# BillyXYB/TransEditor

Hardware: AMD Instinct MI355X
Metric: 256x256 images/sec/GPU, G+D fwd+bwd, batch 16; 1/2/4/8-GPU scaling (higher is better)
Workload: dtype f32

## Files before the change

include/te_hip.h:

```cpp
#ifndef TE_HIP_H
#define TE_HIP_H

#include <stdint.h>

#ifdef __cplusplus
extern "C" {
#endif

#define TE_ABI_VERSION 3

#define TE_ERR_NULL -1
#define TE_ERR_SHAPE -2
#define TE_ERR_UNSUPPORTED -3
#define TE_ERR_WORKSPACE -4

typedef void* te_stream_t;

int te_version(void);
const char* te_last_error_string(void);
const char* te_arch(void);

int te_bias_act_f32(float* out, const float* x, const float* b, const float* ref, int act, int grad,
                    float alpha, float scale, int64_t size_x, int64_t step_b, int64_t size_b,
                    te_stream_t stream);
int te_bias_act_f16(void* out, const void* x, const void* b, const void* ref, int act, int grad,
                    float alpha, float scale, int64_t size_x, int64_t step_b, int64_t size_b,
                    te_stream_t stream);
int te_bias_act_f64(double* out, const double* x, const double* b, const double* ref, int act, int grad,
                    float alpha, float scale, int64_t size_x, int64_t step_b, int64_t size_b,
                    te_stream_t stream);

int64_t te_bias_act_bwd_ws_floats(int64_t outer, int64_t C, int64_t inner);
int te_bias_act_bwd_f32(float* gi, float* gb, float* ws, const float* g, const float* ref, float alpha, float scale,
                        int64_t outer, int64_t C, int64_t inner, te_stream_t stream);
int te_bias_act_bwd_rgb_supported(int64_t outer, int64_t C, int64_t inner);
int te_bias_act_bwd_rgb_f32(float* gi, float* gb, float* ws, const float* g, const float* ref, const float* grgb, const float* wrgb,
                            const float* srgb, float wscale, float alpha, float scale, int64_t outer, int64_t C, int64_t inner,
                            te_stream_t stream);

int te_upfirdn2d_f32(float* out, const float* x, const float* k, int64_t major, int in_h, int in_w,
                     int minor, int kh, int kw, int up_x, int up_y, int down_x, int down_y, int pad_x0,
                     int pad_x1, int pad_y0, int pad_y1, const float* b, int64_t size_b, int act,
                     float alpha, float scale, te_stream_t stream);
int te_upfirdn2d_f16(void* out, const void* x, const void* k, int64_t major, int in_h, int in_w,
                     int minor, int kh, int kw, int up_x, int up_y, int down_x, int down_y, int pad_x0,
                     int pad_x1, int pad_y0, int pad_y1, te_stream_t stream);
int te_upfirdn2d_f64(double* out, const double* x, const double* k, int64_t major, int in_h, int in_w,
                     int minor, int kh, int kw, int up_x, int up_y, int down_x, int down_y, int pad_x0,
                     int pad_x1, int pad_y0, int pad_y1, te_stream_t stream);


#define TE_CONV_3X3 0
#define TE_CONV_T2 1
#define TE_CONV_S2 2
#define TE_CONV_1X1 3
#define TE_CONV_3X3W 4
#define TE_CONV_3X3W6 5

#define TE_CONV_S2S6 6

#define TE_CONV_T2S6 7

#define TE_CONV_1X1S6 8
#define TE_CONV_KINDS 9

#define TE_PACK_FWD 0
#define TE_PACK_DGRAD 1
#define TE_PACK_SWAP 2
#define TE_PACK_WFWD 3
#define TE_PACK_WDGRAD 4
#define TE_PACK_W6FWD 5
#define TE_PACK_W6DGRAD 6
#define TE_PACK_S6FWD 7
#define TE_PACK_S6SWAP 8
#define TE_PACK_T6FWD 9
#define TE_PACK_T6SWAP 10
#define TE_PACK_P6FWD 11
#define TE_PACK_P6DGRAD 12
#define TE_PACK_KINDS 13

int64_t te_conv_packed_numel(int kind_pack, int Co, int Ci, int ksize);
int te_conv_pack_weights_f32(float* wp, const float* w, float wscale, int kind_pack, int Co, int Ci,
                             int ksize, te_stream_t stream);
int te_conv_pack_weights2_f32(float* wp_a, int kind_a, float* wp_b, int kind_b, const float* w, float wscale, int Co, int Ci,
                              int ksize, te_stream_t stream);

int te_conv_pack_weights_multi_f32(int n, float* const* wp, const float* const* w, const float* wscale, const int* kind_pack,
                                   const int* Co, const int* Ci, const int* ksize, te_stream_t stream);

int te_conv_f32(float* out, const float* in, const float* wp, const float* isc, const float* osc,
                const float* bias, int act, int kind, int B, int K, int M, int H, int W,
                te_stream_t stream);
int te_conv_splitk_count(int kind, int B, int K, int M, int H, int W);
int te_conv_wino_supported(int B, int K, int M, int H, int W);
int te_conv_wino6_supported(int B, int K, int M, int H, int W);
int te_conv_s2s6_supported(int B, int K, int M, int H, int W);
int te_conv_t2s6_supported(int B, int K, int M, int H, int W);
int te_conv_p1s6_supported(int B, int K, int M, int H, int W);
int te_conv_wino6_form(int form);
int te_conv_wino6_tiles_per_block(int n);
int te_conv_s2s6_form(int form);
int te_conv_t2s6_form(int form);
int64_t te_conv_t2s6_ws_floats(int B, int K, int H);
int te_conv_ws_f32(float* out, float* ws, const float* in, const float* wp, const float* isc, const float* osc,
                   const float* bias, int act, int kind, int B, int K, int M, int H, int W, te_stream_t stream);
int te_conv_res_f32(float* out, float* ws, const float* in, const float* wp, const float* isc, const float* osc,
                    const float* bias, const float* res, const float* mask_ref, float mask_gain, int act, int kind, int B,
                    int K, int M, int H, int W, te_stream_t stream);

int te_wgrad_slab_count(int kind, int B, int Co, int Ci, int H, int W);
int te_wgrad_pair_form(int kind, int Co, int Ci, int H, int W);
int te_wgrad_split_supported(int kind, int Co, int Ci, int H, int W);
int te_wgrad_split_bf16(int on);
int te_wgrad_t2_wide(int on);
enum { TE_WG6_FP32 = 0, TE_WG6_3X3 = 1, TE_WG6_3X3_PAIR = 2, TE_WG6_T2_WIDE = 3, TE_WG6_T2 = 4, TE_WG6_T2_MASKED = 5, TE_WG6_1X1 = 6 };
int te_wgrad6_form(int kind, int B, int Co, int Ci, int H, int W, int NB);
int te_wgrad_f32(float* slabs, const float* g, const float* x, int kind, int B, int Co, int Ci, int H,
                 int W, int S, te_stream_t stream);
int te_wgrad_group_plan(int kind, int B, int Co, int Ci, int H, int W, int* NB, int* S);
int te_wgrad_group_f32(float* slabs, const float* g, const float* x, int kind, int B, int Co, int Ci, int H, int W, int S, int NB,
                       te_stream_t stream);

int64_t te_wgrad_reduce_ws_floats(int B, int S, int Co, int Ci, int taps, int want_w, int want_isc, int want_osc);
int te_wgrad_reduce_f32(float* gw, float* gisc, float* gosc, float* ws, const float* slabs, const float* w,
                        float wscale, const float* isc, const float* osc, int B, int S, int Co, int Ci,
                        int taps, te_stream_t stream);

int te_rgb_supported(int M, int K, int HW);
int te_rgb_fwd_f32(float* out, const float* x, const float* w, const float* isc, const float* bias, float wscale, int B,
                   int K, int HW, te_stream_t stream);
int te_rgb_dgrad_f32(float* gx, const float* g, const float* w, const float* isc, float wscale, int B, int K, int HW,
                     te_stream_t stream);
int te_rgb_expand_f32(float* out, const float* x3, const float* w, const float* bias, int act, float wscale, int B, int K,
                      int HW, te_stream_t stream);
int te_rgb_wgrad_slab_count(int B, int K, int HW);
int te_rgb_wgrad_f32(float* slabs, const float* g, const float* x, int B, int K, int HW, int S, te_stream_t stream);
int te_rgb_wgrad_sum_f32(float* slabs, const float* g, const float* x, int B, int K, int HW, int S, te_stream_t stream);

int te_attn_fwd_f32(float* o, float* sim, const float* q, const float* k, const float* v, float scale,
                    int N, int G, int M, int L, int D, te_stream_t stream);
int te_attn_bwd_f32(float* gq, float* gk, float* gv, const float* go, const float* gsim_or_null,
                    const float* q, const float* k, const float* v, const float* sim, float scale, int N,
                    int G, int M, int L, int D, te_stream_t stream);

int te_blur_actgrad_tiles(int in_h, int in_w, int kh, int kw, int pad_x0, int pad_x1, int pad_y0, int pad_y1);
int te_blur_actgrad_f32(float* gx, float* partial, const float* g, const float* ref, const float* k, int64_t major, int in_h,
                        int in_w, int kh, int kw, int pad_x0, int pad_x1, int pad_y0, int pad_y1, float alpha, float scale,
                        te_stream_t stream);
int te_blur_gradact_f32(float* gx, float* partial, const float* g, const float* ref, const float* k, int64_t major, int in_h,
                        int in_w, int kh, int kw, int pad_x0, int pad_x1, int pad_y0, int pad_y1, float alpha, float scale,
                        te_stream_t stream);

int te_upfirdn2d_plan(int64_t major, int in_h, int in_w, int minor, int kh, int kw, int up_x, int up_y, int down_x, int down_y,
                      int pad_x0, int pad_x1, int pad_y0, int pad_y1, int* zgroups, int* tiles);
int te_blur_actgrad_plan(int64_t major, int in_h, int in_w, int kh, int kw, int pad_x0, int pad_x1, int pad_y0, int pad_y1,
                         int* zgroups, int* tiles);
int te_blur_gradact_plan(int64_t major, int in_h, int in_w, int kh, int kw, int pad_x0, int pad_x1, int pad_y0, int pad_y1,
                         int* zgroups, int* tiles);
int64_t te_upfirdn2d_direct_cover(int64_t outputs);
int64_t te_chan_scale_cover(int64_t rows, int64_t hw, int aligned16);
int64_t te_bias_act_f32_cover(int64_t size_x, int64_t step_b, int aligned16, int* vec);
int64_t te_bias_act_any_cover(int64_t size_x);
int64_t te_conv_finalize_cover(int64_t outputs);
int64_t te_small_gemm_splitk_finish_cover(int I, int J);
int te_conv_pack_plan(int kind_pack, int Co, int Ci, int ksize, int* blocks, int* tiles);
int te_wgrad_reduce_plan(int B, int S, int Co, int Ci, int taps, int* parts, int64_t* cover);

int te_small_gemm_f32(float* c, float* pre, const float* a, const float* b, const float* bias, const float* residual,
                      float* arowsum, float rs_scale, int I, int J, int K, int64_t sai, int64_t sak, int64_t sbk,
                      int64_t sbj, float alpha, float beta, int act, te_stream_t stream);

int te_small_gemm_splitk_f32(float* c, float* pre, float* ws, int S, const float* a, const float* b, const float* bias,
                             const float* residual, int I, int J, int K, int64_t sai, int64_t sak, int64_t sbk, int64_t sbj,
                             float alpha, float beta, int act, te_stream_t stream);

int te_minibatch_stddev_fwd_f32(float* y, const float* x, int B, int group, int C, int HW, float eps, te_stream_t stream);
int te_minibatch_stddev_bwd_f32(float* gx, const float* gy, const float* x, int B, int group, int C, int HW, float eps,
                                te_stream_t stream);

int te_layer_norm_supported(int64_t R, int N);
int te_layer_norm_fwd_f32(float* y, float* stats, const float* x, int64_t R, int N, float eps, te_stream_t stream);
int te_layer_norm_bwd_f32(float* gx, const float* g, const float* y, const float* stats, int64_t R, int N, te_stream_t stream);

int te_pixel_norm_supported(int64_t B, int D, int C);
int te_pixel_norm_fwd_f32(float* y, float* r, const float* x, int64_t B, int D, int C, float eps, te_stream_t stream);
int te_pixel_norm_bwd_f32(float* gx, const float* g, const float* y, const float* r, int64_t B, int D, int C, te_stream_t stream);

int te_small_gemm_batched_f32(float* c, const float* a, const float* b, const float* bias, int nz, int64_t za, int64_t zc,
                              int64_t zb, int64_t zbias, const int64_t* b_tab, const int64_t* bias_tab, int I, int J, int K,
                              int64_t sai, int64_t sak, int64_t sbk, int64_t sbj, int64_t sci, int64_t scj, float alpha,
                              float beta, int act, te_stream_t stream);

int te_demod_fwd_f32(float* d, float* wsq, const float* w, const float* s, float wscale, float eps, int B, int Co, int Ci,
                     int T, te_stream_t stream);
int te_demod_bwd_f32(float* gw, float* gs, const float* gd, const float* d, const float* w, const float* wsq,
                     const float* s, float wscale, int B, int Co, int Ci, int T, int accumulate, te_stream_t stream);

int te_mt_adam_f32(const int64_t* table, const int32_t* chunks, int n_tensors, int n_chunks, int chunk_elems, double lr,
                   double beta1, double beta2, double eps, int step, te_stream_t stream);
int te_mt_ema_f32(const int64_t* table, const int32_t* chunks, int n_tensors, int n_chunks, int chunk_elems, double decay,
                  te_stream_t stream);

int te_chan_scale_f32(float* out, const float* x, const float* s, int64_t rows, int64_t hw, te_stream_t stream);
int te_chan_dot_f32(float* out, const float* a, const float* b, int64_t rows, int64_t hw, te_stream_t stream);

int te_lpips_stem_fwd_f32(float* out, const float* x, const float* w, const float* b, int N, int H, int W, te_stream_t stream);
int te_lpips_stem_dgrad_f32(float* gx, const float* g, const float* y1, const float* w, int N, int H, int W, te_stream_t stream);
int te_maxpool2_fwd_f32(float* out, const float* x, int64_t planes, int H, int W, te_stream_t stream);
int te_maxpool2_bwd_f32(float* gx, const float* g, const float* x, int64_t planes, int H, int W, te_stream_t stream);
int te_lpips_normalize_f32(float* out, const float* x, int N, int C, int64_t HW, te_stream_t stream);
int te_lpips_head_blocks(int64_t HW);
int te_lpips_head_fwd_f32(float* partial, const float* f, const float* t, const float* w, int N, int Nt, int C, int64_t HW,
                          te_stream_t stream);
int te_lpips_dist_f32(float* d, const float* const* partial, const int64_t* hw, int L, int N, te_stream_t stream);
int te_lpips_head_bwd_f32(float* gf, const float* gin, const float* gd, const float* f, const float* t, const float* w, int N, int Nt,
                          int C, int64_t HW, int relu_mask, te_stream_t stream);
int te_lpips_pair_head_fwd_f32(float* partial, const float* f, const float* w, int N, int C, int64_t HW, te_stream_t stream);
int te_crop_resize_bilinear_f32(float* out, const float* img, int B, int H, int W, int y0, int x0, int hc, int wc, int h, int w,
                                te_stream_t stream);

int64_t te_noise_reg_ws_floats(const int* sizes, int n, int B);
int te_noise_reg_fwd_f32(float* loss, float* ws, float* const* maps, const int* sizes, int n, int B, te_stream_t stream);
int te_noise_reg_bwd_f32(float* const* grads, float* tws, const float* gloss, const float* ws, float* const* maps, const int* sizes,
                         int n, int B, te_stream_t stream);
int te_noise_normalize_f32(float* const* maps, const int* sizes, int n, int B, te_stream_t stream);

int64_t te_prdc_ws_bytes(int N, int M, int D, int k);
int te_row_sqnorm_f32(float* out, const float* x, int N, int D, te_stream_t stream);
int te_prdc_knn_f32(float* r2, const float* x, const float* nx, int N, int D, int k, void* ws, te_stream_t stream);
int te_prdc_counts_f32(int32_t* col_count, int32_t* row_any, float* row_min, const float* x, const float* nx, const float* rr2,
                       const float* y, const float* ny, const float* rf2, int N, int M, int D, void* ws, te_stream_t stream);

int te_vgg_stem_fwd_f32(float* out, const float* x, const float* w, const float* b, int N, int H, int W, te_stream_t stream);
int te_adaptive_avgpool_f32(float* out, const float* x, int64_t planes, int H, int W, int OH, int OW, te_stream_t stream);
int te_fc_stream_splits(int J, int K);
int64_t te_fc_stream_ws_bytes(int64_t I, int J, int K);
int te_fc_stream_f32(float* c, float* ws, const float* a, const float* w, const float* bias, int64_t I, int J, int K, int act,
                     te_stream_t stream);

int64_t te_fid_moments_ws_bytes(int64_t N, int D);
int te_fid_moments_f64(double* S, double* s, void* ws, const float* x, int64_t N, int D, int accumulate, te_stream_t stream);
int te_fid_finalize_f64(double* mean, double* cov, const double* S, const double* s, int64_t n, int D, te_stream_t stream);

int te_gram_f32(float* K, const float* x, int n, int D, te_stream_t stream);
int te_svm_smo_f64(double* alpha, double* rho, int32_t* info, const float* K, const int8_t* y, int n, double C, double eps,
                   int64_t max_iter, te_stream_t stream);
int te_svm_coef_f32(float* w, const float* x, const double* alpha, const int8_t* y, int n, int D, te_stream_t stream);

int te_conv2d_f32(float* out, const float* x, const float* w, const float* bias, int B, int Ci, int Co, int H, int W, int kh, int kw,
                  int s, int py, int px, int Ctot, int c0, int act, te_stream_t stream);
int te_pool3_f32(float* out, const float* x, int B, int C, int H, int W, int mode, int Ctot, int c0, te_stream_t stream);
int te_resize_bilinear_f32(float* out, const float* x, int64_t planes, int H, int W, int OH, int OW, te_stream_t stream);

int te_dex_stem_fwd_f32(float* out, const float* img, const float* w, const float* b, int N, int H, int W, int crop, te_stream_t stream);
int te_cls_score_f32(float* score, float* prob, const float* a, const float* w, const float* bias, int64_t I, int C, int K, int mode,
                     te_stream_t stream);

int te_attr_stem_fwd_f32(float* out, const float* img, const float* w, const float* b, int N, int S, int R, int C0, int preprocessed,
                         te_stream_t stream);
int te_avgpool2_act_f32(float* out, const float* x, int64_t planes, int H, int W, float slope, te_stream_t stream);
int te_attr_score_f32(float* logit, float* score, const float* a, const float* w, const float* bias, int64_t I, int K, float slope,
                      te_stream_t stream);

int te_conv2d_res_f32(float* out, const float* x, const float* w, const float* bias, const float* res, int B, int Ci, int Co, int H, int W,
                      int kh, int kw, int s, int py, int px, int act, te_stream_t stream);
int te_pose_stem_fwd_f32(float* out, const float* img, const float* w, const float* b, int N, int H, int W, int crop, int Co,
                         int preprocessed, te_stream_t stream);
int te_maxpool3s2p1_f32(float* out, const float* x, int64_t planes, int H, int W, te_stream_t stream);

int te_alex_stem_fwd_f32(float* out, const float* x, const float* w, const float* b, int N, int H, int W, int Co, te_stream_t stream);
int te_lpips_unit_f32(float* out, const float* f, int N, int C, int64_t HW, te_stream_t stream);
int64_t te_lpips_allpairs_ws_floats(int N, int C, int64_t HW);
int te_lpips_allpairs_fwd_f32(float* partial, const float* fh, const float* w, int N, int C, int64_t HW, te_stream_t stream);
int te_lpips_allpairs_dist_f32(float* D, const float* const* partial, const int* c, const int64_t* hw, int L, int N, te_stream_t stream);

int te_conv2d_prelu_f32(float* out, const float* x, const float* w, const float* bias, const float* slope, const float* in_scale,
                        const float* in_shift, int B, int Ci, int Co, int H, int W, int kh, int kw, int s, int py, int px, te_stream_t stream);
int te_id_stem_fwd_f32(float* out, const float* img, const float* w, const float* b, const float* slope, int N, int H, int W, int y0, int y1,
                       int x0, int x1, int Pn, int Co, te_stream_t stream);
int te_se_excite_f32(float* gate, const float* pooled, const float* w1, const float* w2, int B, int C, int R, te_stream_t stream);
int te_se_scale_add_f32(float* out, const float* res, const float* gate, const float* sc, int B, int C, int Ho, int Wo, int Hs, int Ws, int s,
                        te_stream_t stream);
int te_rows_unit_f32(float* out, const float* a, int64_t I, int D, te_stream_t stream);
int te_rows_dot_f32(float* out, const float* a, const float* b, int64_t I, int D, te_stream_t stream);

int te_conv2d_prelu_keep_f32(float* out, float* pre, const float* x, const float* w, const float* bias, const float* slope,
                             const float* in_scale, const float* in_shift, int B, int Ci, int Co, int H, int W, int kh, int kw, int s, int py,
                             int px, te_stream_t stream);
int te_id_stem_keep_f32(float* out, float* pre, const float* img, const float* w, const float* b, const float* slope, int N, int H, int W,
                        int y0, int y1, int x0, int x1, int Pn, int Co, te_stream_t stream);
int te_conv2d_dgrad_f32(float* gx, const float* g, const float* wt, const float* pre, const float* slope, const float* in_scale,
                        const float* add, int B, int Ci, int Co, int H, int W, int kh, int kw, int s, int py, int px, int add_s,
                        te_stream_t stream);
int te_se_bwd_f32(float* gr, float* ws, const float* gout, const float* r, const float* gate, const float* pooled, const float* w1,
                  const float* w2, int B, int C, int R, int Ho, int Wo, te_stream_t stream);
int te_id_stem_bwd_f32(float* gimg, float* ws, const float* g, const float* wt, const float* pre, const float* slope, int N, int H, int W,
                       int y0, int y1, int x0, int x1, int Pn, int Co, te_stream_t stream);
int te_rows_unit_bwd_f32(float* ga, const float* ge, const float* e, const float* a, int64_t I, int D, te_stream_t stream);

int te_conv2d_heads_splits(int Ci, int kh, int kw, int Ho, int Wo);
int64_t te_conv2d_heads_ws_bytes(int64_t B, int G, int Cg, int Ci, int kh, int kw, int Ho, int Wo);
int te_conv2d_heads_f32(float* out, float* ws, int64_t ws_bytes, const float* x, const float* w, const float* bias, int B, int G, int Ci,
                        int Cg, int H, int W, int kh, int kw, int s, int py, int px, int Ctot, int c0, int shared, float slope, int splits,
                        te_stream_t stream);
int te_upsample_add_f32(float* out, const float* x, const float* y, int64_t planes, int h, int w, int H, int W, te_stream_t stream);
int te_psp_codes_f32(float* z, float* p, const float* lat, const float* A, const float* bz, const float* z_avg, const float* p_avg,
                     int64_t B, int Ns, int Np, int D, int T, te_stream_t stream);

#ifdef __cplusplus
}
#endif
#endif
```

transeditor_amd/_lib.py:

```python
import ctypes as C
import os

import torch

from . import _abi

_HERE = os.path.dirname(os.path.abspath(__file__))
LIB_PATH = os.path.join(_HERE, 'libte_hip.so')
HEADER_PATH = os.path.join(_HERE, '..', 'include', 'te_hip.h')
_lib = _protos = None

CONV_3X3, CONV_T2, CONV_S2, CONV_1X1, CONV_3X3W, CONV_3X3W6, CONV_S2S6, CONV_T2S6, CONV_1X1S6 = 0, 1, 2, 3, 4, 5, 6, 7, 8
(PACK_FWD, PACK_DGRAD, PACK_SWAP, PACK_WFWD, PACK_WDGRAD, PACK_W6FWD, PACK_W6DGRAD, PACK_S6FWD, PACK_S6SWAP, PACK_T6FWD,
 PACK_T6SWAP, PACK_P6FWD, PACK_P6DGRAD) = range(13)


def _header_text():
    if not os.path.exists(HEADER_PATH):
        raise RuntimeError(f'{HEADER_PATH} is missing: the bindings of libte_hip.so are read from it')
    with open(HEADER_PATH) as f:
        return f.read()


def _prototypes():
    global _protos
    if _protos is None:
        text = _header_text()
        _protos = _abi.parse(text), _abi.abi_version(text)
    return _protos


def __getattr__(name):
    if name == 'EXPORTS':
        return tuple(_prototypes()[0])
    raise AttributeError(f'module {__name__!r} has no attribute {name!r}')


def lib():
    global _lib
    if _lib is None:
        if not os.path.exists(LIB_PATH):
            raise RuntimeError(f'{LIB_PATH} is missing: build it with `python -m transeditor_amd.build` '
                               '(there is no CPU / PyTorch fallback for the TransEditor hot path)')
        protos, version = _prototypes()
        L = C.CDLL(LIB_PATH)
        for name, (res, args) in protos.items():
            if not hasattr(L, name):
                raise RuntimeError(f'{LIB_PATH} does not export {name}')
            fn = getattr(L, name)
            fn.restype, fn.argtypes = res, args
        if L.te_arch() != b'gfx950':
            raise RuntimeError('libte_hip.so was not built for gfx950')
        if L.te_version() != version:
            raise RuntimeError(f'{LIB_PATH} has ABI version {L.te_version()} but include/te_hip.h declares {version}: '
                               'a stale library, rebuild it with `python -m transeditor_amd.build`')
        _lib = L
    return _lib


def _check(rc, what):
    if rc != 0:
        raise RuntimeError(f'{what} failed (code {rc}): {lib().te_last_error_string().decode()}')


def _launch(name, *args):
    rc = getattr(_lib or lib(), name)(*args, _stream())
    if rc:
        _check(rc, name)


_OPS = []


def _op(fn):
    _OPS.append(fn)
    return fn


_cur_dev = getattr(torch._C, '_cuda_getDevice', torch.cuda.current_device)


def _on_current_device(t):
    if t.device.index != _cur_dev():
        raise RuntimeError(f'te_hip: tensor on {t.device} but the current device is cuda:{torch.cuda.current_device()}; '
                           f'call torch.cuda.set_device (one process per GPU) or wrap the call in torch.cuda.device(...)')


def _ptr(t, dtype=torch.float32, dense=True):
    if t is None:
        return None
    if not (t.is_cuda and t.dtype == dtype and (t.is_contiguous() or not dense)):
        name = 'fp32' if dtype == torch.float32 else dtype
        raise RuntimeError(f'te_hip: expected {"a contiguous" if dense else "an"} {name} tensor on the GPU, got {t.dtype} {t.device} '
                           + (f'contiguous={t.is_contiguous()} ' if dense else '') + '(no CPU path exists)')
    _on_current_device(t)
    return t.data_ptr()


_ptr_as = _ptr


def _raw(t):
    return _ptr(t, dense=False)


def _stream():
    return torch.cuda.current_stream().cuda_stream


def _aligned16(t):
    if t is None or t.data_ptr() % 16 == 0:
        return t
    return t.clone(memory_format=torch.contiguous_format)


_OTHER = {torch.float16: 'f16', torch.float64: 'f64'}


def _dispatch(x):
    return (_OTHER[x.dtype], x.dtype) if x.dtype in _OTHER else ('f32', torch.float32)


def _inner(shape):
    n = 1
    for d in shape[2:]:
        n *= d
    return n


@_op
def bias_act(x, b, ref, act, grad, alpha, scale):
    x = x.contiguous()
    sfx, dt = _dispatch(x)
    out = torch.empty_like(x)
    _launch('te_bias_act_' + sfx, _ptr(out, dt), _ptr(x, dt), _ptr(b, dt), _ptr(ref, dt), act, grad, alpha, scale, x.numel(),
            _inner(x.shape), b.numel() if b is not None else 1)
    return out


def _bias_grad_buffers(want_bias, outer, Cn, inner, device):
    if not want_bias:
        return None, None
    n = lib().te_bias_act_bwd_ws_floats(outer, Cn, inner)
    return (torch.empty(Cn, device=device, dtype=torch.float32),
            torch.empty(n, device=device, dtype=torch.float32) if n > 0 else None)


@_op
def bias_act_bwd(g, ref, alpha, scale, want_bias=True):
    g = g.contiguous()
    if g.dtype in _OTHER:
        gi = bias_act(g, None, ref, 3, 1, alpha, scale)
        return gi, (gi.sum(dim=[0] + list(range(2, gi.ndim))) if want_bias else None)
    gi = torch.empty_like(g)
    Cn, inner = g.shape[1], _inner(g.shape)
    gb, ws = _bias_grad_buffers(want_bias, g.shape[0], Cn, inner, g.device)
    _launch('te_bias_act_bwd_f32', _ptr(gi), _ptr(gb), _ptr(ws), _ptr(g), _ptr(ref), alpha, scale, g.shape[0], Cn, inner)
    return gi, gb


def bias_act_bwd_rgb_supported(shape):
    return bool(lib().te_bias_act_bwd_rgb_supported(shape[0], shape[1], _inner(shape)))


@_op
def bias_act_bwd_rgb(g, ref, grgb, wrgb, srgb, wscale, alpha, scale, want_bias=True):
    ref, grgb = _aligned16(ref.contiguous()), _aligned16(grgb.contiguous())
    g = _aligned16(g.contiguous()) if g is not None else None
    gi = torch.empty_like(ref)
    Cn, inner = ref.shape[1], _inner(ref.shape)
    gb, ws = _bias_grad_buffers(want_bias, ref.shape[0], Cn, inner, ref.device)
    _launch('te_bias_act_bwd_rgb_f32', _ptr(gi), _ptr(gb), _ptr(ws), _ptr(g), _ptr(ref), _ptr(grgb), _ptr(wrgb.contiguous()),
            _ptr(srgb.contiguous()) if srgb is not None else None, wscale, alpha, scale, ref.shape[0], Cn, inner)
    return gi, gb


@_op
def upfirdn2d_raw(x, k, up, down, pad, bias=None, act=0, alpha=0.2, scale=1.0):
    x = x.contiguous()
    B, Cn, H, W = x.shape
    kh, kw = k.shape
    px0, px1, py0, py1 = pad
    oh = (H * up[1] + py0 + py1 - kh) // down[1] + 1
    ow = (W * up[0] + px0 + px1 - kw) // down[0] + 1
    if oh <= 0 or ow <= 0:
        raise RuntimeError(f'upfirdn2d: empty output {oh}x{ow}')
    out = torch.empty(B, Cn, oh, ow, device=x.device, dtype=x.dtype)
    sfx, dt = _dispatch(x)
    if sfx != 'f32':
        if bias is not None or act:
            raise RuntimeError('upfirdn2d: the fused bias / activation epilogue exists in fp32 only')
        k = k.to(dt)
    args = [_ptr(out, dt), _ptr(x, dt), _ptr(k.contiguous(), dt), B * Cn, H, W, 1, kh, kw, up[0], up[1], down[0], down[1],
            px0, px1, py0, py1]
    if sfx == 'f32':
        args += [_ptr(bias), bias.numel() if bias is not None else 1, act, alpha, scale]
    _launch('te_upfirdn2d_' + sfx, *args)
    return out


@_op
def blur_actgrad(g, ref, k_flipped, pad, alpha, scale):
    g, ref = g.contiguous(), ref.contiguous()
    B, Cn, H, W = g.shape
    kh, kw = k_flipped.shape
    px0, px1, py0, py1 = pad
    tiles = lib().te_blur_actgrad_tiles(H, W, kh, kw, px0, px1, py0, py1)
    if tiles <= 0:
        raise RuntimeError(f'te_blur_actgrad_tiles failed ({tiles})')
    gx = torch.empty(B, Cn, H + py0 + py1 - kh + 1, W + px0 + px1 - kw + 1, device=g.device, dtype=g.dtype)
    partial = torch.empty(B, Cn, tiles, device=g.device, dtype=g.dtype)
    _launch('te_blur_actgrad_f32', _ptr(gx), _ptr(partial), _ptr(g), _ptr(ref), _ptr(k_flipped.contiguous()), B * Cn, H, W, kh, kw, px0,
            px1, py0, py1, alpha, scale)
    return gx, partial.sum(dim=(0, 2))


@_op
def blur_gradact(g, ref, k_flipped, pad, alpha, scale):
    g, ref = g.contiguous(), ref.contiguous()
    B, Cn, H, W = g.shape
    kh, kw = k_flipped.shape
    px0, px1, py0, py1 = pad
    oh, ow = H + py0 + py1 - kh + 1, W + px0 + px1 - kw + 1
    if tuple(ref.shape) != (B, Cn, oh, ow):
        raise RuntimeError(f'blur_gradact: ref {tuple(ref.shape)} is not the shape of the adjoint blur output {(B, Cn, oh, ow)}')
    tiles = lib().te_blur_actgrad_tiles(H, W, kh, kw, px0, px1, py0, py1)
    if tiles <= 0:
        raise RuntimeError(f'te_blur_actgrad_tiles failed ({tiles})')
    gx = torch.empty(B, Cn, oh, ow, device=g.device, dtype=g.dtype)
    partial = torch.empty(B, Cn, tiles, device=g.device, dtype=g.dtype)
    _launch('te_blur_gradact_f32', _ptr(gx), _ptr(partial), _ptr(g), _ptr(ref), _ptr(k_flipped.contiguous()), B * Cn, H, W, kh, kw, px0,
            px1, py0, py1, alpha, scale)
    return gx, partial.sum(dim=(0, 2))


@_op
def conv_pack(w, kind_pack, wscale=1.0):
    w = w.contiguous()
    Co, Ci, ks, _ = w.shape
    n = lib().te_conv_packed_numel(kind_pack, Co, Ci, ks)
    wp = torch.empty(n, device=w.device, dtype=w.dtype)
    _launch('te_conv_pack_weights_f32', _ptr(wp), _ptr(w), wscale, kind_pack, Co, Ci, ks)
    return wp


@_op
def conv_pack2(w, kind_a, kind_b, wscale=1.0):
    w = w.contiguous()
    Co, Ci, ks, _ = w.shape
    wa = torch.empty(lib().te_conv_packed_numel(kind_a, Co, Ci, ks), device=w.device, dtype=w.dtype)
    wb = torch.empty(lib().te_conv_packed_numel(kind_b, Co, Ci, ks), device=w.device, dtype=w.dtype)
    _launch('te_conv_pack_weights2_f32', _ptr(wa), kind_a, _ptr(wb), kind_b, _ptr(w), wscale, Co, Ci, ks)
    return wa, wb


@_op
def conv_pack_multi(jobs):
    n = len(jobs)
    if not n:
        return
    for wp, w, _, _ in jobs:
        if not (w.is_contiguous() and wp.is_contiguous()):
            raise RuntimeError('te_hip: conv_pack_multi needs dense weights and buffers')
    arr = lambda ty, vals: (ty * n)(*vals)
    _launch('te_conv_pack_weights_multi_f32', n, arr(C.c_void_p, [_ptr(j[0]) for j in jobs]), arr(C.c_void_p, [_ptr(j[1]) for j in jobs]),
            arr(C.c_float, [float(j[3]) for j in jobs]), arr(C.c_int, [int(j[2]) for j in jobs]),
            arr(C.c_int, [j[1].shape[0] for j in jobs]), arr(C.c_int, [j[1].shape[1] for j in jobs]),
            arr(C.c_int, [j[1].shape[2] for j in jobs]))


def wino_ok(B, K, M, H, W):
    return bool(lib().te_conv_wino_supported(B, K, M, H, W))


def s2s6_ok(B, K, M, H, W):
    return bool(lib().te_conv_s2s6_supported(B, K, M, H, W))


def t2s6_ok(B, K, M, H, W):
    return bool(lib().te_conv_t2s6_supported(B, K, M, H, W))


def p1s6_ok(B, K, M, H, W):
    return bool(lib().te_conv_p1s6_supported(B, K, M, H, W))


def wino6_form(form=-1):
    return int(lib().te_conv_wino6_form(form))


def wino6_tiles_per_block(n=-1):
    return int(lib().te_conv_wino6_tiles_per_block(n))


def s2s6_form(form=-1):
    return int(lib().te_conv_s2s6_form(form))


def t2s6_form(form=-1):
    return int(lib().te_conv_t2s6_form(form))


def wino6_ok(B, K, M, H, W):
    return bool(lib().te_conv_wino6_supported(B, K, M, H, W))


def conv_out_shape(kind, B, M, H, W):
    if kind in (CONV_T2, CONV_T2S6):
        return (B, M, 2 * H + 1, 2 * W + 1)
    return (B, M, H, W)


@_op
def conv(x, wp, kind, M, H, W, isc=None, osc=None, bias=None, act=0, res=None, mask_ref=None, mask_gain=1.0):
    x = x.contiguous()
    if kind == CONV_1X1S6:
        x = _aligned16(x)
    res = _aligned16(res.contiguous()) if res is not None else None
    mask_ref = _aligned16(mask_ref.contiguous()) if mask_ref is not None else None
    B, K = x.shape[0], x.shape[1]
    out = torch.empty(conv_out_shape(kind, B, M, H, W), device=x.device, dtype=x.dtype)
    if res is not None and tuple(res.shape) != tuple(out.shape):
        raise RuntimeError(f'te_hip: residual {tuple(res.shape)} does not match the convolution output {tuple(out.shape)}')
    if mask_ref is not None and tuple(mask_ref.shape) != tuple(out.shape):
        raise RuntimeError(f'te_hip: mask reference {tuple(mask_ref.shape)} does not match the convolution output {tuple(out.shape)}')
    S = lib().te_conv_splitk_count(kind, B, K, M, H, W)
    if S < 1:
        raise RuntimeError(f'te_conv_splitk_count failed ({S})')
    ws = torch.empty((S,) + tuple(out.shape), device=x.device, dtype=x.dtype) if S > 1 else None
    if kind == CONV_T2S6:
        ws = torch.empty(B * K * H, device=x.device, dtype=x.dtype)
    _launch('te_conv_res_f32', _ptr(out), _ptr(ws), _ptr(x), _ptr(wp), _ptr(isc), _ptr(osc), _ptr(bias), _ptr(res), _ptr(mask_ref),
            mask_gain, act, kind, B, K, M, H, W)
    return out


@_op
def wgrad_slabs(g, x, kind, H, W, group=False):
    g, x = g.contiguous(), x.contiguous()
    B, Co, Ci = g.shape[0], g.shape[1], x.shape[1]
    taps = 1 if kind == CONV_1X1 else 9
    if group:
        nb, sc = C.c_int(0), C.c_int(0)
        _check(lib().te_wgrad_group_plan(kind, B, Co, Ci, H, W, C.byref(nb), C.byref(sc)), 'te_wgrad_group_plan')
        if nb.value > 1:
            slabs = torch.empty(B // nb.value, sc.value, Co, Ci, taps, device=g.device, dtype=g.dtype)
            _launch('te_wgrad_group_f32', _ptr(slabs), _ptr(g), _ptr(x), kind, B, Co, Ci, H, W, sc.value, nb.value)
            return slabs
    S = lib().te_wgrad_slab_count(kind, B, Co, Ci, H, W)
    if S <= 0:
        raise RuntimeError(f'te_wgrad_slab_count failed ({S})')
    slabs = torch.empty(B, S, Co, Ci, taps, device=g.device, dtype=g.dtype)
    _launch('te_wgrad_f32', _ptr(slabs), _ptr(g), _ptr(x), kind, B, Co, Ci, H, W, S)
    return slabs


def wgrad_t2_wide(on=-1):
    return int(lib().te_wgrad_t2_wide(on))


def wgrad_split(on=-1):
    return int(lib().te_wgrad_split_bf16(on))


def wgrad_split_ok(kind, Co, Ci, H, W):
    return bool(lib().te_wgrad_split_supported(kind, Co, Ci, H, W))


WGRAD6_FORMS = ('fp32', 'w6', 'w6pair', 't2wide', 't2narrow', 't2masked', 'p1')


def wgrad6_form(kind, B, Co, Ci, H, W, NB=1):
    return WGRAD6_FORMS[lib().te_wgrad6_form(kind, B, Co, Ci, H, W, NB)]


def wgrad_pair_form(kind, Co, Ci, H, W):
    return bool(lib().te_wgrad_pair_form(kind, Co, Ci, H, W))


@_op
def wgrad_reduce(slabs, w, wscale=1.0, isc=None, osc=None, want_w=True, want_isc=False, want_osc=False):
    B, S, Co, Ci, taps = slabs.shape
    dev, dt = slabs.device, slabs.dtype
    gw = torch.empty(Co, Ci, taps, device=dev, dtype=dt) if want_w else None
    gisc = torch.empty(B, Ci, device=dev, dtype=dt) if want_isc else None
    gosc = torch.empty(B, Co, device=dev, dtype=dt) if want_osc else None
    n = lib().te_wgrad_reduce_ws_floats(B, S, Co, Ci, taps, int(want_w), int(want_isc), int(want_osc))
    if n < 0:
        raise RuntimeError(f'te_wgrad_reduce_ws_floats failed ({n})')
    ws = torch.empty(n, device=dev, dtype=dt) if n > 0 else None
    _launch('te_wgrad_reduce_f32', _ptr(gw), _ptr(gisc), _ptr(gosc), _ptr(ws), _ptr(slabs), _ptr(w.contiguous()), wscale, _ptr(isc),
            _ptr(osc), B, S, Co, Ci, taps)
    return gw, gisc, gosc


def rgb_supported(M, K, HW):
    return bool(lib().te_rgb_supported(M, K, HW))


@_op
def rgb_fwd(x, w, isc, bias, wscale=1.0):
    x = _aligned16(x.contiguous())
    B, K, H, W = x.shape
    out = torch.empty(B, 3, H, W, device=x.device, dtype=x.dtype)
    _launch('te_rgb_fwd_f32', _ptr(out), _ptr(x), _ptr(w.contiguous()), _ptr(isc), _ptr(bias), wscale, B, K, H * W)
    return out


@_op
def rgb_dgrad(g, w, isc, K, wscale=1.0):
    g = _aligned16(g.contiguous())
    B, _, H, W = g.shape
    gx = torch.empty(B, K, H, W, device=g.device, dtype=g.dtype)
    _launch('te_rgb_dgrad_f32', _ptr(gx), _ptr(g), _ptr(w.contiguous()), _ptr(isc), wscale, B, K, H * W)
    return gx


@_op
def rgb_wgrad_sum_slabs(g3, x):
    g3, x = g3.contiguous(), x.contiguous()
    B, K, H, W = x.shape
    S = lib().te_rgb_wgrad_slab_count(B, K, H * W)
    slabs = torch.empty(B, S, 4, K, device=x.device, dtype=x.dtype)
    _launch('te_rgb_wgrad_sum_f32', _ptr(slabs), _ptr(g3), _ptr(x), B, K, H * W, S)
    return slabs


@_op
def rgb_expand(x3, w3k, bias, act, wscale=1.0):
    x3 = _aligned16(x3.contiguous())
    B, _, H, W = x3.shape
    K = w3k.shape[1]
    out = torch.empty(B, K, H, W, device=x3.device, dtype=x3.dtype)
    _launch('te_rgb_expand_f32', _ptr(out), _ptr(x3), _ptr(w3k.contiguous()), _ptr(bias), act, wscale, B, K, H * W)
    return out


@_op
def rgb_wgrad_slabs(g, x):
    g, x = g.contiguous(), x.contiguous()
    B, K, H, W = x.shape
    S = lib().te_rgb_wgrad_slab_count(B, K, H * W)
    slabs = torch.empty(B, S, 3, K, 1, device=x.device, dtype=x.dtype)
    _launch('te_rgb_wgrad_f32', _ptr(slabs), _ptr(g), _ptr(x), B, K, H * W, S)
    return slabs


@_op
def small_gemm(I, J, K, a, sai, sak, b, sbk, sbj, bias=None, residual=None, alpha=1.0, beta=1.0, act=0, want_pre=False,
               rowsum_scale=None):
    c = torch.empty(I, J, device=a.device, dtype=a.dtype)
    pre = torch.empty_like(c) if want_pre else None
    rs = torch.empty(I, device=a.device, dtype=a.dtype) if rowsum_scale is not None else None
    _launch('te_small_gemm_f32', _ptr(c), _ptr(pre), _raw(a), _raw(b), _ptr(bias), _ptr(residual), _ptr(rs),
            rowsum_scale if rowsum_scale is not None else 0.0, I, J, K, sai, sak, sbk, sbj, alpha, beta, act)
    return c, pre, rs


@_op
def small_gemm_splitk(I, J, K, S, a, sai, sak, b, sbk, sbj, bias=None, residual=None, alpha=1.0, beta=1.0, act=0, want_pre=False):
    c = torch.empty(I, J, device=a.device, dtype=a.dtype)
    pre = torch.empty_like(c) if want_pre else None
    ws = torch.empty(S, I, J, device=a.device, dtype=a.dtype)
    _launch('te_small_gemm_splitk_f32', _ptr(c), _ptr(pre), _ptr(ws), S, _raw(a), _raw(b), _ptr(bias), _ptr(residual), I, J, K, sai, sak,
            sbk, sbj, alpha, beta, act)
    return c, pre


@_op
def minibatch_stddev_fwd(x, group, eps, chunks=1):
    x = x.contiguous()
    B, Cn, H, W = x.shape
    y = torch.empty(B, Cn + 1, H, W, device=x.device, dtype=x.dtype)
    Bc = B // chunks
    for c in range(chunks):
        _launch('te_minibatch_stddev_fwd_f32', _ptr(y[c * Bc:(c + 1) * Bc]), _ptr(x[c * Bc:(c + 1) * Bc]), Bc, group, Cn, H * W, eps)
    return y


@_op
def minibatch_stddev_bwd(gy, x, group, eps, chunks=1):
    gy = gy.contiguous()
    B, Cn, H, W = x.shape
    gx = torch.empty_like(x)
    Bc = B // chunks
    for c in range(chunks):
        sl = slice(c * Bc, (c + 1) * Bc)
        _launch('te_minibatch_stddev_bwd_f32', _ptr(gx[sl]), _ptr(gy[sl]), _ptr(x[sl]), Bc, group, Cn, H * W, eps)
    return gx


@_op
def small_gemm_batched(c, a, b, bias, nz, za, zc, I, J, K, sai, sak, sbk, sbj, sci, scj, zb=0, zbias=0, b_tab=None,
                       bias_tab=None, alpha=1.0, beta=1.0, act=0):
    bt = (C.c_int64 * nz)(*b_tab) if b_tab is not None else None
    bit = (C.c_int64 * nz)(*bias_tab) if bias_tab is not None else None
    _launch('te_small_gemm_batched_f32', _raw(c), _raw(a), _raw(b), _raw(bias), nz, za, zc, zb, zbias, bt, bit, I, J, K, sai, sak, sbk, sbj,
            sci, scj, alpha, beta, act)
    return c


def layer_norm_supported(R, N):
    return bool(lib().te_layer_norm_supported(R, N))


@_op
def layer_norm_fwd(x2, eps):
    R, N = x2.shape
    y = torch.empty_like(x2)
    stats = torch.empty(R, 2, device=x2.device, dtype=x2.dtype)
    _launch('te_layer_norm_fwd_f32', _ptr(y), _ptr(stats), _ptr(x2), R, N, eps)
    return y, stats


@_op
def layer_norm_bwd(g2, y2, stats):
    R, N = y2.shape
    gx = torch.empty_like(y2)
    _launch('te_layer_norm_bwd_f32', _ptr(gx), _ptr(g2), _ptr(y2), _ptr(stats), R, N)
    return gx


def pixel_norm_supported(B, D, Cn):
    return bool(lib().te_pixel_norm_supported(B, D, Cn))


@_op
def pixel_norm_fwd(x, eps):
    B, D, Cn = x.shape
    y = torch.empty_like(x)
    r = torch.empty(B, Cn, device=x.device, dtype=x.dtype)
    _launch('te_pixel_norm_fwd_f32', _ptr(y), _ptr(r), _ptr(x), B, D, Cn, eps)
    return y, r


@_op
def pixel_norm_bwd(g, y, r):
    B, D, Cn = y.shape
    gx = torch.empty_like(y)
    _launch('te_pixel_norm_bwd_f32', _ptr(gx), _ptr(g), _ptr(y), _ptr(r), B, D, Cn)
    return gx


@_op
def demod_fwd(w, s, wscale, eps):
    Co, Ci, T = w.shape
    B = s.shape[0]
    d = torch.empty(B, Co, device=w.device, dtype=w.dtype)
    wsq = torch.empty(Co, Ci, device=w.device, dtype=w.dtype)
    _launch('te_demod_fwd_f32', _ptr(d), _ptr(wsq), _ptr(w), _ptr(s), wscale, eps, B, Co, Ci, T)
    return d, wsq


@_op
def demod_from_wsq(wsq, s, eps):
    Co, Ci = wsq.shape
    B = s.shape[0]
    d = torch.empty(B, Co, device=wsq.device, dtype=wsq.dtype)
    _launch('te_demod_fwd_f32', _ptr(d), None, _ptr(wsq), _ptr(s), 1.0, eps, B, Co, Ci, 0)
    return d


@_op
def demod_bwd(gd, d, w, wsq, s, wscale, want_w=True, want_s=True, into=None):
    Co, Ci, T = w.shape
    B = s.shape[0]
    if into is not None:
        gw, gs = into
    else:
        gw = torch.empty_like(w) if want_w else None
        gs = torch.empty_like(s) if want_s else None
    _launch('te_demod_bwd_f32', _ptr(gw), _ptr(gs), _ptr(gd.contiguous()), _ptr(d), _ptr(w), _ptr(wsq), _ptr(s), wscale, B, Co, Ci, T,
            1 if into is not None else 0)
    return gw, gs


@_op
def attn_fwd(q, k, v, scale, groups):
    q, k, v = q.contiguous(), k.contiguous(), v.contiguous()
    N, M, Cn = q.shape
    L = k.shape[1]
    D = Cn // groups
    o = torch.empty_like(q)
    sim = torch.empty(N, groups, M, L, device=q.device, dtype=q.dtype)
    _launch('te_attn_fwd_f32', _ptr(o), _ptr(sim), _ptr(q), _ptr(k), _ptr(v), scale, N, groups, M, L, D)
    return o, sim


@_op
def attn_bwd(go, gsim, q, k, v, sim, scale, groups):
    N, M, Cn = q.shape
    L = k.shape[1]
    gq, gk, gv = torch.empty_like(q), torch.empty_like(k), torch.empty_like(v)
    _launch('te_attn_bwd_f32', _ptr(gq), _ptr(gk), _ptr(gv), _ptr(go.contiguous()), _ptr(gsim.contiguous()) if gsim is not None else None,
            _ptr(q), _ptr(k), _ptr(v), _ptr(sim), scale, N, groups, M, L, Cn // groups)
    return gq, gk, gv


@_op
def mt_adam(table, chunks, n_tensors, n_chunks, chunk_elems, lr, beta1, beta2, eps, step):
    _on_current_device(table)
    _launch('te_mt_adam_f32', table.data_ptr(), chunks.data_ptr(), n_tensors, n_chunks, chunk_elems, lr, beta1, beta2, eps, step)


@_op
def mt_ema(table, chunks, n_tensors, n_chunks, chunk_elems, decay):
    _on_current_device(table)
    _launch('te_mt_ema_f32', table.data_ptr(), chunks.data_ptr(), n_tensors, n_chunks, chunk_elems, float(decay))


@_op
def chan_scale(x, s):
    x, s = x.contiguous(), s.contiguous()
    rows = x.shape[0] * x.shape[1]
    out = torch.empty_like(x)
    _launch('te_chan_scale_f32', _ptr(out), _ptr(x), _ptr(s), rows, x.numel() // max(rows, 1))
    return out


@_op
def chan_dot(a, b):
    a, b = a.contiguous(), b.contiguous()
    rows = a.shape[0] * a.shape[1]
    out = torch.empty(a.shape[0], a.shape[1], device=a.device, dtype=a.dtype)
    _launch('te_chan_dot_f32', _ptr(out), _ptr(a), _ptr(b), rows, a.numel() // max(rows, 1))
    return out


@_op
def lpips_stem_fwd(x, w, b):
    x = x.contiguous()
    N, _, H, W = x.shape
    out = torch.empty(N, 64, H, W, device=x.device, dtype=x.dtype)
    _launch('te_lpips_stem_fwd_f32', _ptr(out), _ptr(x), _ptr(w), _ptr(b), N, H, W)
    return out


@_op
def lpips_stem_dgrad(g, y1, w):
    g = g.contiguous()
    N, _, H, W = g.shape
    gx = torch.empty(N, 3, H, W, device=g.device, dtype=g.dtype)
    _launch('te_lpips_stem_dgrad_f32', _ptr(gx), _ptr(g), _ptr(y1), _ptr(w), N, H, W)
    return gx


@_op
def maxpool2_fwd(x):
    x = x.contiguous()
    N, Cn, H, W = x.shape
    out = torch.empty(N, Cn, H // 2, W // 2, device=x.device, dtype=x.dtype)
    _launch('te_maxpool2_fwd_f32', _ptr(out), _ptr(x), N * Cn, H, W)
    return out


@_op
def maxpool2_bwd(g, x):
    g = g.contiguous()
    N, Cn, H, W = x.shape
    gx = torch.empty_like(x)
    _launch('te_maxpool2_bwd_f32', _ptr(gx), _ptr(g), _ptr(x), N * Cn, H, W)
    return gx


@_op
def lpips_normalize(x):
    x = x.contiguous()
    out = torch.empty_like(x)
    _launch('te_lpips_normalize_f32', _ptr(out), _ptr(x), x.shape[0], x.shape[1], x.shape[2] * x.shape[3])
    return out


@_op
def lpips_head_fwd(f, t_hat, w):
    f = f.contiguous()
    N, Cn, H, W = f.shape
    nb = lib().te_lpips_head_blocks(H * W)
    partial = torch.empty(N, nb, device=f.device, dtype=f.dtype)
    _launch('te_lpips_head_fwd_f32', _ptr(partial), _ptr(f), _ptr(t_hat), _ptr(w), N, t_hat.shape[0], Cn, H * W)
    return partial


@_op
def lpips_dist(partials, hws):
    L, N = len(partials), partials[0].shape[0]
    d = torch.empty(N, device=partials[0].device, dtype=torch.float32)
    ptrs = (C.c_void_p * L)(*[_ptr(p) for p in partials])
    hw = (C.c_int64 * L)(*hws)
    _launch('te_lpips_dist_f32', _ptr(d), ptrs, hw, L, N)
    return d


@_op
def lpips_head_bwd(gd, f, t_hat, w, gin=None, relu_mask=True):
    f = f.contiguous()
    N, Cn, H, W = f.shape
    gf = torch.empty_like(f)
    _launch('te_lpips_head_bwd_f32', _ptr(gf), _ptr(gin.contiguous()) if gin is not None else None, _ptr(gd.contiguous()), _ptr(f),
            _ptr(t_hat), _ptr(w), N, t_hat.shape[0], Cn, H * W, 1 if relu_mask else 0)
    return gf


@_op
def lpips_pair_head_fwd(f, w):
    if f.shape[0] % 2:
        raise RuntimeError(f'te_hip: the paired LPIPS head needs an even batch, got {f.shape[0]}')
    f = f.contiguous()
    N, Cn, H, W = f.shape[0] // 2, f.shape[1], f.shape[2], f.shape[3]
# ... 642 lines not shown
```

transeditor_amd/csrc/bias_act.hip:

```cpp
#include "te_common.h"
#include <hip/hip_fp16.h>

namespace {

__device__ __forceinline__ float act_one(float x, float r, int mode, float alpha) {
    switch (mode) {
        case 30: return x > 0.f ? x : x * alpha;
        case 31: return r > 0.f ? x : x * alpha;
        case 12:
        case 32: return 0.f;
        default: return x;
    }
}

__global__ __launch_bounds__(256) void bias_act_vec4_kernel(float4* __restrict__ out, const float4* __restrict__ x,
                                                            const float* __restrict__ b, const float4* __restrict__ ref,
                                                            int mode, float alpha, float scale, uint32_t n4,
                                                            uint32_t step_b4, uint32_t size_b) {
    const uint32_t stride = gridDim.x * blockDim.x;
    for (uint32_t i = blockIdx.x * blockDim.x + threadIdx.x; i < n4; i += stride) {
        float4 v = x[i];
        if (b) {
            const float bb = b[(i / step_b4) % size_b];
            v.x += bb; v.y += bb; v.z += bb; v.w += bb;
        }
        float4 r = make_float4(0.f, 0.f, 0.f, 0.f);
        if (ref) r = ref[i];
        float4 y;
        y.x = act_one(v.x, r.x, mode, alpha) * scale;
        y.y = act_one(v.y, r.y, mode, alpha) * scale;
        y.z = act_one(v.z, r.z, mode, alpha) * scale;
        y.w = act_one(v.w, r.w, mode, alpha) * scale;
        out[i] = y;
    }
}

__global__ __launch_bounds__(256) void bias_act_scalar_kernel(float* __restrict__ out, const float* __restrict__ x,
                                                              const float* __restrict__ b, const float* __restrict__ ref,
                                                              int mode, float alpha, float scale, int64_t n,
                                                              int64_t step_b, int64_t size_b) {
    const int64_t stride = (int64_t)gridDim.x * blockDim.x;
    for (int64_t i = (int64_t)blockIdx.x * blockDim.x + threadIdx.x; i < n; i += stride) {
        float v = x[i];
        if (b) v += b[(i / step_b) % size_b];
        const float r = ref ? ref[i] : 0.f;
        out[i] = act_one(v, r, mode, alpha) * scale;
    }
}

__device__ __forceinline__ float wave_sum(float v) {
#pragma unroll
    for (int off = 32; off > 0; off >>= 1) v += __shfl_down(v, off, 64);
    return v;
}

__device__ __forceinline__ float block_sum_256(float v, float* lds4) {
    v = wave_sum(v);
    const int lane = threadIdx.x & 63, wid = threadIdx.x >> 6;
    if (lane == 0) lds4[wid] = v;
    __syncthreads();
    return lds4[0] + lds4[1] + lds4[2] + lds4[3];
}

constexpr int kBwdVecPerThread = 4;
__global__ __launch_bounds__(256) void bias_act_bwd_rows_kernel(float4* __restrict__ gi, float* __restrict__ part,
                                                                const float4* __restrict__ g, const float4* __restrict__ ref,
                                                                float alpha, float scale, uint32_t C, uint32_t inner4) {
    __shared__ float lds4[4];
    const uint32_t c = blockIdx.y, n = blockIdx.z;
    const size_t row = ((size_t)n * C + c) * inner4;
    const uint32_t base = blockIdx.x * (256 * kBwdVecPerThread);
    float acc = 0.f;
#pragma unroll
    for (int it = 0; it < kBwdVecPerThread; ++it) {
        const uint32_t i = base + it * 256 + threadIdx.x;
        if (i < inner4) {
            const float4 gv = g[row + i], rv = ref[row + i];
            float4 o;
            o.x = gv.x * (rv.x > 0.f ? 1.f : alpha) * scale;
            o.y = gv.y * (rv.y > 0.f ? 1.f : alpha) * scale;
            o.z = gv.z * (rv.z > 0.f ? 1.f : alpha) * scale;
            o.w = gv.w * (rv.w > 0.f ? 1.f : alpha) * scale;
            gi[row + i] = o;
            acc += (o.x + o.y) + (o.z + o.w);
        }
    }
    if (part) {
        const float tot = block_sum_256(acc, lds4);
        if (threadIdx.x == 0) part[((size_t)c * gridDim.z + n) * gridDim.x + blockIdx.x] = tot;
    }
}

__global__ __launch_bounds__(64) void bias_parts_sum_kernel(float* __restrict__ gb, const float* __restrict__ part, uint32_t parts) {
    const float* p = part + (size_t)blockIdx.x * parts;
    float acc = 0.f;
    for (uint32_t j = threadIdx.x; j < parts; j += 64) acc += p[j];
    acc = wave_sum(acc);
    if (threadIdx.x == 0) gb[blockIdx.x] = acc;
}

__global__ __launch_bounds__(256) void bias_act_bwd_rgb_rows_kernel(float4* __restrict__ gi, float* __restrict__ part,
                                                                    const float4* __restrict__ g, const float4* __restrict__ ref,
                                                                    const float4* __restrict__ grgb, const float* __restrict__ wrgb,
                                                                    const float* __restrict__ srgb, float wscale, float alpha,
                                                                    float scale, uint32_t C, uint32_t inner4) {
    __shared__ float lds4[4];
    const uint32_t c = blockIdx.y, n = blockIdx.z;
    const size_t row = ((size_t)n * C + c) * inner4;
    const size_t rrow = (size_t)n * 3 * inner4;
    const float sc = (srgb ? srgb[(size_t)n * C + c] : 1.f) * wscale;
    const float c0 = sc * wrgb[c], c1 = sc * wrgb[C + c], c2 = sc * wrgb[2 * C + c];
    const uint32_t base = blockIdx.x * (256 * kBwdVecPerThread);
    float acc = 0.f;
#pragma unroll
    for (int it = 0; it < kBwdVecPerThread; ++it) {
        const uint32_t i = base + it * 256 + threadIdx.x;
        if (i < inner4) {
            const float4 rv = ref[row + i];
            const float4 r0 = grgb[rrow + i], r1 = grgb[rrow + inner4 + i], r2 = grgb[rrow + 2 * (size_t)inner4 + i];
            float4 gv = g ? g[row + i] : make_float4(0.f, 0.f, 0.f, 0.f);
            gv.x += c0 * r0.x + c1 * r1.x + c2 * r2.x;
            gv.y += c0 * r0.y + c1 * r1.y + c2 * r2.y;
            gv.z += c0 * r0.z + c1 * r1.z + c2 * r2.z;
            gv.w += c0 * r0.w + c1 * r1.w + c2 * r2.w;
            float4 o;
            o.x = gv.x * (rv.x > 0.f ? 1.f : alpha) * scale;
            o.y = gv.y * (rv.y > 0.f ? 1.f : alpha) * scale;
            o.z = gv.z * (rv.z > 0.f ? 1.f : alpha) * scale;
            o.w = gv.w * (rv.w > 0.f ? 1.f : alpha) * scale;
            gi[row + i] = o;
            acc += (o.x + o.y) + (o.z + o.w);
        }
    }
    if (part) {
        const float tot = block_sum_256(acc, lds4);
        if (threadIdx.x == 0) part[((size_t)c * gridDim.z + n) * gridDim.x + blockIdx.x] = tot;
    }
}

__global__ __launch_bounds__(256) void bias_act_bwd_chan_kernel(float* __restrict__ gi, float* __restrict__ gb,
                                                                const float* __restrict__ g, const float* __restrict__ ref,
                                                                float alpha, float scale, int64_t outer, int64_t C,
                                                                int64_t inner) {
    __shared__ float lds4[4];
    const int64_t c = blockIdx.x;
    const int64_t per = outer * inner;
    float acc = 0.f;
    for (int64_t e = threadIdx.x; e < per; e += 256) {
        const int64_t n = e / inner, i = e - n * inner;
        const int64_t idx = (n * C + c) * inner + i;
        const float o = g[idx] * (ref[idx] > 0.f ? 1.f : alpha) * scale;
        gi[idx] = o;
        acc += o;
    }
    if (gb) {
        const float tot = block_sum_256(acc, lds4);
        if (threadIdx.x == 0) gb[c] = tot;
    }
}

__global__ __launch_bounds__(256) void bias_act_bwd_2d_kernel(float* __restrict__ gi, float* __restrict__ gb,
                                                              const float* __restrict__ g, const float* __restrict__ ref,
                                                              float alpha, float scale, int64_t N, int64_t C) {
    const int64_t c = (int64_t)blockIdx.x * 256 + threadIdx.x;
    if (c >= C) return;
    float acc = 0.f;
    for (int64_t n = 0; n < N; ++n) {
        const int64_t idx = n * C + c;
        const float o = g[idx] * (ref[idx] > 0.f ? 1.f : alpha) * scale;
        gi[idx] = o;
        acc += o;
    }
    if (gb) gb[c] = acc;
}

inline int bias_act_grid(int64_t items) { return (int)std::min<int64_t>(te::cdiv(items, 256), te::kNumCU * 8); }
inline bool bias_act_vec(int64_t size_x, bool has_b, int64_t step_b, bool al16) {
    return (size_x % 4 == 0) && (!has_b || step_b % 4 == 0) && al16 && (size_x / 4 < (int64_t)0xFFFFFFFF);
}

template <typename T> struct AccOf { typedef T type; };
template <> struct AccOf<__half> { typedef float type; };

template <typename T>
__global__ __launch_bounds__(256) void bias_act_any_kernel(T* __restrict__ out, const T* __restrict__ x, const T* __restrict__ b,
                                                           const T* __restrict__ ref, int mode, float alpha_, float scale_,
                                                           int64_t n, int64_t step_b, int64_t size_b) {
    typedef typename AccOf<T>::type A;
    const A alpha = (A)(T)alpha_, scale = (A)(T)scale_;
    const int64_t stride = (int64_t)gridDim.x * blockDim.x;
    for (int64_t i = (int64_t)blockIdx.x * blockDim.x + threadIdx.x; i < n; i += stride) {
        A v = (A)x[i];
        if (b) v += (A)b[(i / step_b) % size_b];
        const A r = ref ? (A)ref[i] : (A)0;
        A y;
        switch (mode) {
            case 30: y = v > (A)0 ? v : v * alpha; break;
            case 31: y = r > (A)0 ? v : v * alpha; break;
            case 12:
            case 32: y = (A)0; break;
            default: y = v;
        }
        out[i] = (T)(y * scale);
    }
}

template <typename T>
int bias_act_any(T* out, const T* x, const T* b, const T* ref, int act, int grad, float alpha, float scale, int64_t size_x,
                 int64_t step_b, int64_t size_b, te_stream_t stream_, const char* what) {
    TE_REQUIRE(out && x, TE_ERR_NULL, "%s: out/x is NULL", what);
    TE_REQUIRE(size_x >= 0, TE_ERR_SHAPE, "%s: size_x < 0", what);
    TE_REQUIRE(!b || (step_b > 0 && size_b > 0), TE_ERR_SHAPE, "%s: bias given but step_b/size_b <= 0", what);
    if (size_x == 0) return 0;
    const int grid = bias_act_grid(size_x);
    bias_act_any_kernel<T><<<grid, 256, 0, (hipStream_t)stream_>>>(out, x, b, ref, act * 10 + grad, alpha, scale, size_x,
                                                                   b ? step_b : 1, b ? size_b : 1);
    return te::launch_status(what);
}

}

extern "C" int te_bias_act_f16(void* out, const void* x, const void* b, const void* ref, int act, int grad, float alpha,
                               float scale, int64_t size_x, int64_t step_b, int64_t size_b, te_stream_t stream) {
    return bias_act_any<__half>((__half*)out, (const __half*)x, (const __half*)b, (const __half*)ref, act, grad, alpha, scale,
                                size_x, step_b, size_b, stream, "te_bias_act_f16");
}

extern "C" int te_bias_act_f64(double* out, const double* x, const double* b, const double* ref, int act, int grad, float alpha,
                               float scale, int64_t size_x, int64_t step_b, int64_t size_b, te_stream_t stream) {
    return bias_act_any<double>(out, x, b, ref, act, grad, alpha, scale, size_x, step_b, size_b, stream, "te_bias_act_f64");
}

extern "C" int te_bias_act_f32(float* out, const float* x, const float* b, const float* ref, int act, int grad,
                               float alpha, float scale, int64_t size_x, int64_t step_b, int64_t size_b,
                               te_stream_t stream_) {
    TE_REQUIRE(out && x, TE_ERR_NULL, "te_bias_act_f32: out/x is NULL");
    TE_REQUIRE(size_x >= 0, TE_ERR_SHAPE, "te_bias_act_f32: size_x < 0");
    TE_REQUIRE(!b || (step_b > 0 && size_b > 0), TE_ERR_SHAPE, "te_bias_act_f32: bias given but step_b/size_b <= 0");
    if (size_x == 0) return 0;
    hipStream_t stream = (hipStream_t)stream_;
    const int mode = act * 10 + grad;
    const bool vec = bias_act_vec(size_x, b != nullptr, step_b, te::aligned16(out) && te::aligned16(x) && (!ref || te::aligned16(ref)));
    if (vec) {
        const uint32_t n4 = (uint32_t)(size_x / 4);
        const int grid = bias_act_grid(n4);
        bias_act_vec4_kernel<<<grid, 256, 0, stream>>>((float4*)out, (const float4*)x, b, (const float4*)ref, mode, alpha,
                                                       scale, n4, b ? (uint32_t)(step_b / 4) : 1u,
                                                       b ? (uint32_t)size_b : 1u);
    } else {
        const int grid = bias_act_grid(size_x);
        bias_act_scalar_kernel<<<grid, 256, 0, stream>>>(out, x, b, ref, mode, alpha, scale, size_x, b ? step_b : 1,
                                                         b ? size_b : 1);
    }
    return te::launch_status("te_bias_act_f32");
}

extern "C" int64_t te_bias_act_f32_cover(int64_t size_x, int64_t step_b, int aligned16_, int* vec_out) {
    if (size_x <= 0 || step_b < 0) return TE_ERR_SHAPE;
    const bool vec = bias_act_vec(size_x, step_b > 0, step_b, aligned16_ != 0);
    if (vec_out) *vec_out = vec ? 1 : 0;
    return (int64_t)bias_act_grid(vec ? size_x / 4 : size_x) * 256 * (vec ? 4 : 1);
}

extern "C" int64_t te_bias_act_any_cover(int64_t size_x) {
    return size_x > 0 ? (int64_t)bias_act_grid(size_x) * 256 : TE_ERR_SHAPE;
}

static bool bwd_rows_path(int64_t outer, int64_t C, int64_t inner) {
    return inner % 4 == 0 && inner >= 1024 && C <= 65535 && outer <= 65535;
}

extern "C" int64_t te_bias_act_bwd_ws_floats(int64_t outer, int64_t C, int64_t inner) {
    if (outer <= 0 || C <= 0 || inner <= 0 || !bwd_rows_path(outer, C, inner)) return 0;
    return C * outer * te::cdiv(inner / 4, 256 * kBwdVecPerThread);
}

extern "C" int te_bias_act_bwd_f32(float* gi, float* gb, float* ws, const float* g, const float* ref, float alpha, float scale,
                                   int64_t outer, int64_t C, int64_t inner, te_stream_t stream_) {
    TE_REQUIRE(gi && g && ref, TE_ERR_NULL, "te_bias_act_bwd_f32: gi/g/ref is NULL");
    TE_REQUIRE(outer >= 0 && C > 0 && inner > 0, TE_ERR_SHAPE, "te_bias_act_bwd_f32: bad dims");
    if (outer == 0) return 0;
    hipStream_t stream = (hipStream_t)stream_;
    if (inner == 1) {
        bias_act_bwd_2d_kernel<<<(int)te::cdiv(C, 256), 256, 0, stream>>>(gi, gb, g, ref, alpha, scale, outer, C);
    } else if (bwd_rows_path(outer, C, inner) && te::aligned16(gi) && te::aligned16(g) && te::aligned16(ref) && (!gb || ws)) {
        const uint32_t inner4 = (uint32_t)(inner / 4);
        dim3 grid((unsigned)te::cdiv(inner4, 256 * kBwdVecPerThread), (unsigned)C, (unsigned)outer);
        bias_act_bwd_rows_kernel<<<grid, 256, 0, stream>>>((float4*)gi, gb ? ws : nullptr, (const float4*)g, (const float4*)ref, alpha,
                                                           scale, (uint32_t)C, inner4);
        if (gb) bias_parts_sum_kernel<<<(int)C, 64, 0, stream>>>(gb, ws, (uint32_t)(grid.x * grid.z));
    } else {
        bias_act_bwd_chan_kernel<<<(int)C, 256, 0, stream>>>(gi, gb, g, ref, alpha, scale, outer, C, inner);
    }
    return te::launch_status("te_bias_act_bwd_f32");
}

extern "C" int te_bias_act_bwd_rgb_supported(int64_t outer, int64_t C, int64_t inner) {
    return (outer > 0 && C > 0 && bwd_rows_path(outer, C, inner)) ? 1 : 0;
}

extern "C" int te_bias_act_bwd_rgb_f32(float* gi, float* gb, float* ws, const float* g, const float* ref, const float* grgb,
                                       const float* wrgb, const float* srgb, float wscale, float alpha, float scale, int64_t outer,
                                       int64_t C, int64_t inner, te_stream_t stream_) {
    TE_REQUIRE(gi && ref && grgb && wrgb, TE_ERR_NULL, "te_bias_act_bwd_rgb_f32: gi/ref/grgb/wrgb is NULL");
    TE_REQUIRE(!gb || ws, TE_ERR_NULL, "te_bias_act_bwd_rgb_f32: the bias gradient needs the workspace (te_bias_act_bwd_ws_floats)");
    TE_REQUIRE(te_bias_act_bwd_rgb_supported(outer, C, inner), TE_ERR_UNSUPPORTED,
               "te_bias_act_bwd_rgb_f32: needs inner %% 4 == 0 and inner >= 1024 (use te_rgb_dgrad_f32 + te_bias_act_bwd_f32)");
    TE_REQUIRE(te::aligned16(gi) && (!g || te::aligned16(g)) && te::aligned16(ref) && te::aligned16(grgb), TE_ERR_UNSUPPORTED,
               "te_bias_act_bwd_rgb_f32: 16-byte aligned tensors required");
    const uint32_t inner4 = (uint32_t)(inner / 4);
    dim3 grid((unsigned)te::cdiv(inner4, 256 * kBwdVecPerThread), (unsigned)C, (unsigned)outer);
    hipStream_t stream = (hipStream_t)stream_;
    bias_act_bwd_rgb_rows_kernel<<<grid, 256, 0, stream>>>((float4*)gi, gb ? ws : nullptr, (const float4*)g, (const float4*)ref,
                                                          (const float4*)grgb, wrgb, srgb, wscale, alpha, scale, (uint32_t)C, inner4);
    if (gb) bias_parts_sum_kernel<<<(int)C, 64, 0, stream>>>(gb, ws, (uint32_t)(grid.x * grid.z));
    return te::launch_status("te_bias_act_bwd_rgb_f32");
}
```

transeditor_amd/csrc/conv_common.h:

```cpp
#pragma once
#include "te_common.h"
#include <stdlib.h>
#include <algorithm>

typedef float f32x16 __attribute__((ext_vector_type(16)));
typedef float f32x4 __attribute__((ext_vector_type(4)));

constexpr unsigned OOBH = 0x40000000u;

__device__ __forceinline__ __amdgpu_buffer_rsrc_t make_rsrc(const float* p, unsigned bytes) {
    return __builtin_amdgcn_make_buffer_rsrc((void*)p, 0, bytes, 0x00020000);
}
__device__ __forceinline__ float buf_load(__amdgpu_buffer_rsrc_t r, unsigned off) {
    return __builtin_bit_cast(float, __builtin_amdgcn_raw_buffer_load_b32(r, off, 0, 0));
}

constexpr int KPAD = 16;
constexpr int MPAD = 128;
constexpr int NTHREADS = 256;


int te_wino_launch(float* out, const float* in, const float* U, const float* isc, const float* osc, const float* bias, const float* res,
                   const float* mask_ref, float mask_gain, int act, int B, int K, int M, int H, int W, hipStream_t s);
int te_wino6_launch(float* out, const float* in, const float* U, const float* isc, const float* osc, const float* bias, const float* res,
                    const float* mask_ref, float mask_gain, int act, int B, int K, int M, int H, int W, hipStream_t s);
int te_s2s6_launch(float* out, const float* in, const float* U, const float* isc, const float* osc, const float* bias, const float* res,
                   const float* mask_ref, float mask_gain, int act, int B, int K, int M, int H, int W, hipStream_t s);
int te_t2s6_launch(float* out, const float* in, const float* U, const float* isc, const float* osc, const float* bias, int act,
                   int B, int K, int M, int H, int W, hipStream_t s, float* colbuf = nullptr);
int te_t2s6_edge_launch(float* out, const float* in, const float* wplain, const float* isc, const float* osc, const float* bias, int act,
                        int B, int K, int M, int H, int W, int Kp, int Mp, hipStream_t s, const float* colbuf = nullptr);
int te_p1s6_launch(float* out, const float* in, const float* U, const float* res, int B, int K, int M, int H, int W, hipStream_t s);
```

transeditor_amd/csrc/rgb.hip:

```cpp
#include "te_common.h"

namespace {

constexpr int KMAX = 512;
constexpr int NOUT = 3;

__global__ __launch_bounds__(256) void rgb_fwd_kernel(float* __restrict__ out, const float* __restrict__ x,
                                                      const float* __restrict__ w, const float* __restrict__ isc,
                                                      const float* __restrict__ bias, float wscale, int K, int HW) {
    __shared__ float ws[NOUT][KMAX];
    const int b = blockIdx.y, tid = threadIdx.x;
    for (int k = tid; k < K; k += 256) {
        const float s = (isc ? isc[(size_t)b * K + k] : 1.f) * wscale;
#pragma unroll
        for (int o = 0; o < NOUT; ++o) ws[o][k] = w[o * K + k] * s;
    }
    __syncthreads();
    const int HW4 = HW >> 2;
    const int p4 = blockIdx.x * 256 + tid;
    if (p4 >= HW4) return;
    const float4* xp = reinterpret_cast<const float4*>(x + (size_t)b * K * HW) + p4;
    float4 acc[NOUT];
#pragma unroll
    for (int o = 0; o < NOUT; ++o) acc[o] = make_float4(0.f, 0.f, 0.f, 0.f);
#pragma unroll 8
    for (int k = 0; k < K; ++k) {
        const float4 v = xp[(size_t)k * HW4];
#pragma unroll
        for (int o = 0; o < NOUT; ++o) {
            const float c = ws[o][k];
            acc[o].x += c * v.x; acc[o].y += c * v.y; acc[o].z += c * v.z; acc[o].w += c * v.w;
        }
    }
#pragma unroll
    for (int o = 0; o < NOUT; ++o) {
        const float bb = bias ? bias[o] : 0.f;
        acc[o].x += bb; acc[o].y += bb; acc[o].z += bb; acc[o].w += bb;
        reinterpret_cast<float4*>(out + ((size_t)b * NOUT + o) * HW)[p4] = acc[o];
    }
}

__global__ __launch_bounds__(256) void rgb_dgrad_kernel(float* __restrict__ gx, const float* __restrict__ g,
                                                        const float* __restrict__ w, const float* __restrict__ isc,
                                                        float wscale, int K, int HW, const float* __restrict__ bias = nullptr,
                                                        int act = 0) {
    __shared__ float ws[NOUT][KMAX];
    const int b = blockIdx.y, tid = threadIdx.x;
    for (int k = tid; k < K; k += 256) {
        const float s = (isc ? isc[(size_t)b * K + k] : 1.f) * wscale;
#pragma unroll
        for (int o = 0; o < NOUT; ++o) ws[o][k] = w[o * K + k] * s;
    }
    __syncthreads();
    const int HW4 = HW >> 2;
    const int p4 = blockIdx.x * 256 + tid;
    if (p4 >= HW4) return;
    float4 gv[NOUT];
#pragma unroll
    for (int o = 0; o < NOUT; ++o) gv[o] = reinterpret_cast<const float4*>(g + ((size_t)b * NOUT + o) * HW)[p4];
    float4* op = reinterpret_cast<float4*>(gx + (size_t)b * K * HW) + p4;
    const float gain = act == 3 ? 1.4142135623730951f : 1.f;
#pragma unroll 4
    for (int k = 0; k < K; ++k) {
        const float c0 = ws[0][k], c1 = ws[1][k], c2 = ws[2][k];
        const float bb = bias ? bias[k] : 0.f;
        float4 r;
        r.x = c0 * gv[0].x + c1 * gv[1].x + c2 * gv[2].x + bb;
        r.y = c0 * gv[0].y + c1 * gv[1].y + c2 * gv[2].y + bb;
        r.z = c0 * gv[0].z + c1 * gv[1].z + c2 * gv[2].z + bb;
        r.w = c0 * gv[0].w + c1 * gv[1].w + c2 * gv[2].w + bb;
        if (act >= 3) {
            r.x = (r.x > 0.f ? r.x : 0.2f * r.x) * gain; r.y = (r.y > 0.f ? r.y : 0.2f * r.y) * gain;
            r.z = (r.z > 0.f ? r.z : 0.2f * r.z) * gain; r.w = (r.w > 0.f ? r.w : 0.2f * r.w) * gain;
        }
        op[(size_t)k * HW4] = r;
    }
}

inline int rgb_pow2(int v) { int p = 1; while (p < v) p <<= 1; return p; }
inline int rgb_tile_px(int K) { return std::max(32, std::min(256, 8192 / rgb_pow2(K))); }

template <bool SUM>
__global__ __launch_bounds__(256) void rgb_wgrad_kernel(float* __restrict__ slabs, const float* __restrict__ g,
                                                        const float* __restrict__ x, int K, int HW, int S, int TPX, int lgTPX, int K2) {
    constexpr int NROW = SUM ? NOUT + 1 : NOUT;
    extern __shared__ __attribute__((aligned(16))) float smem[];
    float* xl = smem;
    float* gl = smem + K * (TPX + 1);
    const int b = blockIdx.y, c = blockIdx.x, tid = threadIdx.x;
    const int ntile = (HW + TPX - 1) / TPX;
    const int t0 = (int)((int64_t)ntile * c / S), t1 = (int)((int64_t)ntile * (c + 1) / S);
    const float* xb = x + (size_t)b * K * HW;
    const float* gb = g + (size_t)b * NOUT * HW;
    const bool vec4 = (HW & 3) == 0 && ((reinterpret_cast<uintptr_t>(x) & 15) == 0);
    const int parts = K2 >= 256 ? 1 : 256 / K2;
    const int kk = K2 >= 256 ? tid : (tid & (K2 - 1)), part = K2 >= 256 ? 0 : tid / K2;
    const int nh = K2 > 256 ? 2 : 1;
    float acc[2][NOUT + 1] = {{0.f, 0.f, 0.f, 0.f}, {0.f, 0.f, 0.f, 0.f}};
    for (int tl = t0; tl < t1; ++tl) {
        const int p0 = tl * TPX;
        __syncthreads();
        if (vec4) {
            for (int e0 = 0; e0 < K * TPX; e0 += 256 * 8 * 4) {
                float4 st[8];
#pragma unroll
                for (int j = 0; j < 8; ++j) {
                    const int e = e0 + 4 * (tid + 256 * j), k = e >> lgTPX, pp = e & (TPX - 1);
                    const bool ok = e < K * TPX && p0 + pp < HW;
                    st[j] = ok ? *reinterpret_cast<const float4*>(xb + (size_t)k * HW + p0 + pp) : make_float4(0.f, 0.f, 0.f, 0.f);
                }
#pragma unroll
                for (int j = 0; j < 8; ++j) {
                    const int e = e0 + 4 * (tid + 256 * j), k = e >> lgTPX, pp = e & (TPX - 1);
                    if (e < K * TPX) {
                        float* d = xl + k * (TPX + 1) + pp;
                        d[0] = st[j].x; d[1] = st[j].y; d[2] = st[j].z; d[3] = st[j].w;
                    }
                }
            }
        } else {
            for (int e0 = 0; e0 < K * TPX; e0 += 256 * 8) {
                float st[8];
#pragma unroll
                for (int j = 0; j < 8; ++j) {
                    const int e = e0 + tid + 256 * j, k = e >> lgTPX, pp = e & (TPX - 1);
                    const bool ok = e < K * TPX && p0 + pp < HW;
                    const float v = xb[ok ? (size_t)k * HW + p0 + pp : 0];
                    st[j] = ok ? v : 0.f;
                }
#pragma unroll
                for (int j = 0; j < 8; ++j) {
                    const int e = e0 + tid + 256 * j, k = e >> lgTPX, pp = e & (TPX - 1);
                    if (e < K * TPX) xl[k * (TPX + 1) + pp] = st[j];
                }
            }
        }
        for (int e = tid; e < NOUT * TPX; e += 256) {
            const int o = e >> lgTPX, pp = e & (TPX - 1);
            gl[e] = (p0 + pp < HW) ? gb[(size_t)o * HW + p0 + pp] : 0.f;
        }
        __syncthreads();
        for (int h = 0; h < nh; ++h) {
            const int k = kk + 256 * h;
            if (k < K) {
#pragma unroll 4
                for (int pp = part; pp < TPX; pp += parts) {
                    const float xv = xl[k * (TPX + 1) + pp];
#pragma unroll
                    for (int o = 0; o < NOUT; ++o) acc[h][o] += gl[o * TPX + pp] * xv;
                    if (SUM) acc[h][NOUT] += xv;
                }
            }
        }
    }
    float* sl = slabs + ((size_t)b * S + c) * NROW * K;
    if (parts > 1) {
        __syncthreads();
        float* red = smem;
#pragma unroll
        for (int o = 0; o < NROW; ++o) red[(part * NROW + o) * K2 + kk] = acc[0][o];
        __syncthreads();
        if (part == 0 && kk < K) {
#pragma unroll
            for (int o = 0; o < NROW; ++o) {
                float a = 0.f;
                for (int q = 0; q < parts; ++q) a += red[(q * NROW + o) * K2 + kk];
                sl[o * K + kk] = a;
            }
        }
        return;
    }
    for (int h = 0; h < nh; ++h) {
        const int k = kk + 256 * h;
        if (k < K) {
#pragma unroll
            for (int o = 0; o < NROW; ++o) sl[o * K + k] = acc[h][o];
        }
    }
}

inline bool ok_shape(int K, int HW) { return K > 0 && K <= KMAX && HW > 0 && (HW & 3) == 0; }

}

extern "C" int te_rgb_supported(int M, int K, int HW) { return (M == NOUT && ok_shape(K, HW)) ? 1 : 0; }

extern "C" int te_rgb_fwd_f32(float* out, const float* x, const float* w, const float* isc, const float* bias, float wscale,
                              int B, int K, int HW, te_stream_t stream_) {
    TE_REQUIRE(out && x && w, TE_ERR_NULL, "te_rgb_fwd_f32: NULL pointer");
    TE_REQUIRE(B > 0 && ok_shape(K, HW), TE_ERR_UNSUPPORTED, "te_rgb_fwd_f32: need K <= 512 and H*W %% 4 == 0");
    dim3 grid((unsigned)te::cdiv(HW / 4, 256), (unsigned)B);
    rgb_fwd_kernel<<<grid, 256, 0, (hipStream_t)stream_>>>(out, x, w, isc, bias, wscale, K, HW);
    return te::launch_status("te_rgb_fwd_f32");
}

extern "C" int te_rgb_dgrad_f32(float* gx, const float* g, const float* w, const float* isc, float wscale, int B, int K,
                                int HW, te_stream_t stream_) {
    TE_REQUIRE(gx && g && w, TE_ERR_NULL, "te_rgb_dgrad_f32: NULL pointer");
    TE_REQUIRE(B > 0 && ok_shape(K, HW), TE_ERR_UNSUPPORTED, "te_rgb_dgrad_f32: need K <= 512 and H*W %% 4 == 0");
    dim3 grid((unsigned)te::cdiv(HW / 4, 256), (unsigned)B);
    rgb_dgrad_kernel<<<grid, 256, 0, (hipStream_t)stream_>>>(gx, g, w, isc, wscale, K, HW);
    return te::launch_status("te_rgb_dgrad_f32");
}

extern "C" int te_rgb_expand_f32(float* out, const float* x3, const float* w, const float* bias, int act, float wscale, int B,
                                 int K, int HW, te_stream_t stream_) {
    TE_REQUIRE(out && x3 && w, TE_ERR_NULL, "te_rgb_expand_f32: NULL pointer");
    TE_REQUIRE(B > 0 && ok_shape(K, HW), TE_ERR_UNSUPPORTED, "te_rgb_expand_f32: need K <= 512 and H*W %% 4 == 0");
    TE_REQUIRE(act == 0 || act == 3 || act == 4, TE_ERR_UNSUPPORTED, "te_rgb_expand_f32: act must be 0, 3 or 4");
    dim3 grid((unsigned)te::cdiv(HW / 4, 256), (unsigned)B);
    rgb_dgrad_kernel<<<grid, 256, 0, (hipStream_t)stream_>>>(out, x3, w, nullptr, wscale, K, HW, bias, act);
    return te::launch_status("te_rgb_expand_f32");
}

extern "C" int te_rgb_wgrad_slab_count(int B, int K, int HW) {
    if (B <= 0 || K <= 0 || HW <= 0) return TE_ERR_SHAPE;
    const int64_t ntile = te::cdiv(HW, rgb_tile_px(K));
    int64_t S = te::cdiv(4 * te::kNumCU, B);
    return (int)std::max<int64_t>(1, std::min<int64_t>(S, ntile));
}

extern "C" int te_rgb_wgrad_f32(float* slabs, const float* g, const float* x, int B, int K, int HW, int S, te_stream_t stream_) {
    TE_REQUIRE(slabs && g && x, TE_ERR_NULL, "te_rgb_wgrad_f32: NULL pointer");
    TE_REQUIRE(B > 0 && K > 0 && K <= KMAX && HW > 0 && S > 0, TE_ERR_UNSUPPORTED, "te_rgb_wgrad_f32: need 0 < K <= 512");
    const int TPX = rgb_tile_px(K), K2 = rgb_pow2(K);
    int lg = 0;
    while ((1 << lg) < TPX) ++lg;
    const size_t lds = sizeof(float) * std::max<size_t>((size_t)K * (TPX + 1) + NOUT * TPX, (size_t)256 * (NOUT + 1));
    static std::atomic<uint64_t> attr_done{0};
    te::allow_big_lds(attr_done, (const void*)rgb_wgrad_kernel<false>, 96 * 1024);
    dim3 grid((unsigned)S, (unsigned)B);
    rgb_wgrad_kernel<false><<<grid, 256, lds, (hipStream_t)stream_>>>(slabs, g, x, K, HW, S, TPX, lg, K2);
    return te::launch_status("te_rgb_wgrad_f32");
}

extern "C" int te_rgb_wgrad_sum_f32(float* slabs, const float* g, const float* x, int B, int K, int HW, int S, te_stream_t stream_) {
    TE_REQUIRE(slabs && g && x, TE_ERR_NULL, "te_rgb_wgrad_sum_f32: NULL pointer");
    TE_REQUIRE(B > 0 && K > 0 && K <= KMAX && HW > 0 && S > 0, TE_ERR_UNSUPPORTED, "te_rgb_wgrad_sum_f32: need 0 < K <= 512");
    const int TPX = rgb_tile_px(K), K2 = rgb_pow2(K);
    int lg = 0;
    while ((1 << lg) < TPX) ++lg;
    const size_t lds = sizeof(float) * std::max<size_t>((size_t)K * (TPX + 1) + NOUT * TPX, (size_t)256 * (NOUT + 1));
    static std::atomic<uint64_t> attr_done{0};
    te::allow_big_lds(attr_done, (const void*)rgb_wgrad_kernel<true>, 96 * 1024);
    dim3 grid((unsigned)S, (unsigned)B);
    rgb_wgrad_kernel<true><<<grid, 256, lds, (hipStream_t)stream_>>>(slabs, g, x, K, HW, S, TPX, lg, K2);
    return te::launch_status("te_rgb_wgrad_sum_f32");
}
```

transeditor_amd/csrc/wino6.hip:

```cpp
#include "split6_common.h"
#include "wino6_schedule.h"
#ifdef W6P_PROF
#define TE_PROF
#endif
#include "te_prof.h"

namespace {

constexpr int WT = 512, KC = 16, TW = 32, NP = TW / 2, BM = 64, TH = 8;
constexpr int U_CHUNKS = 36 * 2 * 64;

struct Wino6Args {
    float* out; const float* in; const u32x4* U; const float* isc; const float* osc; const float* bias; const float* res;
    const float* mref; float mgain; int act;
    int B, K, M, H, W, ntiles, mblocks, tiles_x, tiles_y, nt8;
    int lists;
    int lgpw;
};

constexpr int PH = 4, PR = PH + 2;
constexpr int TP_PLANE = PR * 2 * NP * 4;
constexpr int TP_DWORDS = 12 * TP_PLANE;
constexpr int GT = WT / 2;
constexpr int P_IN = (PR * NP * 8) / GT;
static_assert(PR * NP * 8 == P_IN * GT, "items must divide over the group");

PROF_BUFFER(w6p, 2048 * 8 * 8)
constexpr int SLOT0 = 21;

template <bool ISC>
__global__ __launch_bounds__(WT, 2) void wino6p_kernel(const Wino6Args p) {
    extern __shared__ __attribute__((aligned(16))) unsigned char smem_raw[];
    u32x4* ul = reinterpret_cast<u32x4*>(smem_raw);
    const int tid = threadIdx.x, lane = tid & 63, l31 = lane & 31, half = lane >> 5;
    const int wid = __builtin_amdgcn_readfirstlane(tid >> 6);
    const int grp = wid >> 2, wq = wid & 3, wm = wq >> 1, wrl = wq & 1, gt = tid & (GT - 1);
    unsigned* tl = reinterpret_cast<unsigned*>(smem_raw + U_CHUNKS * 16) + grp * TP_DWORDS;
    const u32x4* tl4 = reinterpret_cast<const u32x4*>(tl);
    int tile, mb;
    if (!split6_tile(p.ntiles, p.nt8, p.mblocks, tile, mb)) return;
    const int pwm = (1 << p.lgpw) - 1;
    const int tx = tile % p.tiles_x, ty = (tile / p.tiles_x) % p.tiles_y, b = (tile / (p.tiles_x * p.tiles_y)) << (4 - p.lgpw);
    const int x0 = tx * TW, y0 = ty * TH, yh = y0 + PH * grp;
    const float* inb = p.in + (size_t)b * p.K * p.H * p.W;
    const float* iscb = ISC ? p.isc + (size_t)b * p.K : nullptr;
    const bool has_left = x0 == 0, has_right = x0 + TW >= p.W, has_rowout = (yh == 0) || (yh + PH == p.H);

    f32x16 acc[4];
#pragma unroll
    for (int c = 0; c < 4; ++c)
#pragma unroll
        for (int r = 0; r < 16; ++r) acc[c][r] = 0.f;

    unsigned g_off[P_IN];
    int l_off[P_IN], e_flag[P_IN];
#pragma unroll
    for (int i = 0; i < P_IN; ++i) {
        const int e = gt + GT * i;
        const int jj = e & 15, q = (e >> 4) & 7, row = e >> 7;
        const int gy = yh - 1 + row;
        const int sj = jj >> p.lgpw, jl = jj & pwm;
        const bool left = x0 == 0 && jl == 0, right = x0 + TW >= p.W && jl == pwm, rowout = gy < 0 || gy >= p.H;
        e_flag[i] = (left ? 1 : 0) | (right ? 2 : 0) | (rowout ? 4 : 0);
        const int gyc = gy < 0 ? 0 : (gy >= p.H ? p.H - 1 : gy);
        g_off[i] = (unsigned)(sj * p.K * p.H * p.W + (2 * q * p.H + gyc) * p.W + x0 + 2 * jl - 1 + (left ? 1 : 0) - (right ? 1 : 0));
        l_off[i] = ((row * 2 + (q >> 2)) * NP + jj) * 4 + (q & 3);
    }
    const unsigned q2 = 2u * ((gt >> 4) & 7) + (unsigned)(((gt & 15) >> p.lgpw) * p.K);
    const size_t plane = (size_t)p.H * p.W;
    const int MT = p.M >> 5;
    f32x4 rin[P_IN][2];
    f32x2 rsc = {1.f, 1.f};
    const int nstage = p.K / KC;
    auto fetch_scales = [&](int s) {
        if (ISC) rsc = *reinterpret_cast<const f32x2u*>(iscb + s * KC + q2);
    };
    auto fetch_item = [&](int i, int s) {
#pragma unroll
        for (int h2 = 0; h2 < 2; ++h2)
            rin[i][h2] = *reinterpret_cast<const f32x4u*>(inb + ((size_t)s * KC + h2) * plane + g_off[i]);
    };
    auto issue = [&](int s) {
        fetch_scales(s);
#pragma unroll
        for (int i = 0; i < P_IN; ++i) fetch_item(i, s);
    };
    auto issue_u = [&](int uh, int s) {
        const u32x4* us = p.U + (size_t)s * 36 * MT * 64;
#pragma unroll
        for (int r = 0; r < 9; ++r) {
            const int j = wq * 9 + r, piece = j / 12, rem = j % 12, kc = (rem >> 1) + 6 * uh, mt = rem & 1;
            const int pk = piece * 12 + kc;
            const u32x4* g = us + ((size_t)pk * MT + 2 * mb + mt) * 64 + (unsigned)lane;
            __builtin_amdgcn_global_load_lds((const __attribute__((address_space(1))) void*)g,
                                             (__attribute__((address_space(3))) void*)(ul + (pk * 2 + mt) * 64), 16, 0, 0);
        }
    };
    unsigned res[P_IN][4][3];
    float te = 0.f, to = 0.f, fe = 0.f, fo = 0.f;
    constexpr int N_SLOT = 3 + 4 * 4 * P_IN;
    auto arith = [&](int k) {
        if (k < 0) {
        } else if (k < P_IN) {
#pragma unroll
            for (int h2 = 0; h2 < 2; ++h2) {
                f32x4 v = rin[k][h2];
                const int f = e_flag[k];
                if (has_left) {
                    asm volatile("" ::: "memory");
                    if (f & 1) { v[3] = v[2]; v[2] = v[1]; v[1] = v[0]; v[0] = 0.f; }
                }
                if (has_right) {
                    asm volatile("" ::: "memory");
                    if (f & 2) { v[0] = v[1]; v[1] = v[2]; v[2] = v[3]; v[3] = 0.f; }
                }
                if (has_rowout) {
                    asm volatile("" ::: "memory");
                    if (f & 4) { v[0] = 0.f; v[1] = 0.f; v[2] = 0.f; v[3] = 0.f; }
                }
                rin[k][h2] = ISC ? v * rsc[h2] : v;
                asm volatile("" : "+v"(rin[k][h2]));
            }
        } else if (k < N_SLOT) {
            const int u = (k - P_IN) >> 2, j = (k - P_IN) & 3, i = u >> 2, c = u & 3;
            float ve = 0.f, vo = 0.f;
            if (j == 0) {
                const f32x4 e = rin[i][0], o = rin[i][1];
                ve = c == 0 ? e[0] - e[2] : (c == 1 ? e[1] + e[2] : (c == 2 ? e[2] - e[1] : e[1] - e[3]));
                vo = c == 0 ? o[0] - o[2] : (c == 1 ? o[1] + o[2] : (c == 2 ? o[2] - o[1] : o[1] - o[3]));
            }
            split6_step4(j, ve, vo, te, to, fe, fo, res[i][c][0], res[i][c][1], res[i][c][2]);
        }
    };
    auto write_res = [&]() {
#pragma unroll
        for (int i = 0; i < P_IN; ++i)
#pragma unroll
            for (int c = 0; c < 4; ++c)
#pragma unroll
                for (int pc = 0; pc < 3; ++pc) tl[l_off[i] + (pc * 4 + c) * TP_PLANE] = res[i][c][pc];
    };
    const int rr = l31 >> 4, jj = l31 & 15;
    const int b_chunk = ((2 * wrl + rr) * 2 + half) * NP + jj;
    const int a_chunk = wm * 64 + lane;

    issue(0);
    if (grp == 0) { issue_u(0, 0); issue_u(1, 0); }
#pragma unroll
    for (int k = 0; k < N_SLOT; ++k) arith(k);
    write_res();
    issue(1);
    if (grp == 0) {
        if (ISC) asm volatile("s_waitcnt vmcnt(7)" ::: "memory");
        else asm volatile("s_waitcnt vmcnt(6)" ::: "memory");
    }
    split6_barrier();
    const int nphase = 2 * nstage;
    PROF_ONLY(unsigned long long pc[8] = {0, 0, 0, 0, 0, 0, 0, 0};)
    PROF_ONLY(const unsigned long long pstart = __builtin_readcyclecounter(), rstart = __builtin_amdgcn_s_memrealtime();)
    for (int ph = 0; ph < nphase; ++ph) {
        const bool last = ph == nphase - 1;
        PROF_T(t0);
        if ((ph & 1) == grp) {
            bf16x8 av[2][3], bv[2][3];
            const int fs2 = min((ph >> 1) + 2, nstage - 1);
            auto rd1 = [&](int g, int slot, int q) {
                const int ky = g >> 2, c = g & 3;
                if (q < 3) av[slot][q] = __builtin_bit_cast(bf16x8, ul[a_chunk + ((q * 3 + ky) * 4 + c) * 128]);
                else bv[slot][q - 3] = __builtin_bit_cast(bf16x8, tl4[b_chunk + (((q - 3) * 4 + c) * PR + ky) * 2 * NP]);
            };
#pragma unroll
            for (int q = 0; q < 6; ++q) rd1(0, 0, q);
            __builtin_amdgcn_s_setprio(1);
#pragma unroll
            for (int g = 0; g < 12; ++g) {
                const int slot = g & 1, c = g & 3;
                if (g == 5) { PROF_T(ta); split6_barrier(); PROF_T(tb); PROF_ACC(pc[0], t0, ta); PROF_ACC(pc[1], ta, tb); PROF_ONLY(pc[2] -= tb;) }
                __builtin_amdgcn_sched_barrier(0);
#pragma unroll
                for (int q = 0; q < 6; ++q) {
                    split6_product(q, av[slot], bv[slot], acc[c], acc[c]);
                    if (g + 1 < 12 && q < 3) { rd1(g + 1, slot ^ 1, 2 * q); rd1(g + 1, slot ^ 1, 2 * q + 1); }
                    arith(g * 6 + q - SLOT0);
                    {
                        constexpr int LASTQ = 71 - SLOT0;
                        const int k = g * 6 + q - SLOT0;
                        if (k == P_IN - 1) fetch_scales(fs2);
#pragma unroll
                        for (int i = 0; i < P_IN; ++i)
                            if (k == (P_IN + 16 * i + 12 < LASTQ ? P_IN + 16 * i + 12 : LASTQ)) fetch_item(i, fs2);
                    }
                    __builtin_amdgcn_sched_barrier(0);
                }
            }
            __builtin_amdgcn_s_setprio(0);
            PROF_ONLY({ asm volatile("s_nop 0" ::: "memory"); PROF_T(tc); pc[2] += tc; })
        } else {
            const int cs = (ph + 1) >> 1;
            const bool work = cs >= 1 && cs < nstage;
            if (grp == 1 && work) issue_u(1, cs);
            __builtin_amdgcn_sched_barrier(0);
            write_res();
            if (grp == 1 && work) split6_wait_vm();
            PROF_T(ta);
            split6_barrier();
            PROF_T(tb);
            if (grp == 0 && work) {
                issue_u(0, cs);
                split6_wait_vm();
            }
            PROF_T(tc);
            PROF_ACC(pc[3], t0, ta); PROF_ACC(pc[4], ta, tb); PROF_ACC(pc[5], tb, tc);
        }
        PROF_T(t8);
        if (!last) split6_barrier();
        PROF_T(t9);
        PROF_ACC(pc[6], t8, t9);
    }
    PROF_ONLY(if (lane == 0 && blockIdx.x < 2048) {
        unsigned long long* d = te_w6p_prof_buf + ((size_t)blockIdx.x * 8 + wid) * 8;
        _Pragma("unroll")
        for (int i = 0; i < 6; ++i) d[i] = pc[i];
        d[6] = pc[6] | ((__builtin_amdgcn_s_memrealtime() - rstart) << 40);
        d[7] = ((unsigned long long)nstage << 48) | ((__builtin_readcyclecounter() - pstart) & 0xFFFFFFFFFFFFull);
    })
    const int wr = grp * 2 + wrl;
    const int mbase = mb * BM + wm * 32;
    const int bo = b + (jj >> p.lgpw);
    const size_t off0 = ((size_t)bo * p.M + mbase) * plane + (size_t)(y0 + 2 * wr + rr) * p.W + x0 + 2 * (jj & pwm);
    const float g_pos = p.act == 3 ? 1.4142135623730951f : 1.f;
    float scv[16], biv[16];
#pragma unroll
    for (int r = 0; r < 16; ++r) {
        const int m = mbase + (r & 3) + 8 * (r >> 2) + 4 * half;
        scv[r] = p.osc ? p.osc[(size_t)bo * p.M + m] : 1.f;
        biv[r] = p.bias ? p.bias[m] : 0.f;
    }
    f32x2 resv[16], mrefv[16];
    if (p.res) {
#pragma unroll
        for (int r = 0; r < 16; ++r)
            resv[r] = *reinterpret_cast<const f32x2*>(p.res + off0 + (size_t)((r & 3) + 8 * (r >> 2) + 4 * half) * plane);
    }
    if (p.mref) {
#pragma unroll
        for (int r = 0; r < 16; ++r)
            mrefv[r] = *reinterpret_cast<const f32x2*>(p.mref + off0 + (size_t)((r & 3) + 8 * (r >> 2) + 4 * half) * plane);
    }
#pragma unroll
    for (int r = 0; r < 16; ++r) {
        const int dm = (r & 3) + 8 * (r >> 2) + 4 * half;
        float v0 = acc[0][r] + acc[1][r] + acc[2][r];
        float v1 = acc[1][r] - acc[2][r] - acc[3][r];
        const float sc = scv[r], bi = biv[r];
        v0 = v0 * sc + bi;
        v1 = v1 * sc + bi;
        if (p.act >= 3) {
            v0 = (v0 > 0.f ? v0 : v0 * 0.2f) * g_pos;
            v1 = (v1 > 0.f ? v1 : v1 * 0.2f) * g_pos;
        }
        const size_t o = off0 + (size_t)dm * plane;
        if (p.res) { v0 += resv[r][0]; v1 += resv[r][1]; }
        if (p.mref) {
            v0 *= mrefv[r][0] > 0.f ? p.mgain : 0.2f * p.mgain;
            v1 *= mrefv[r][1] > 0.f ? p.mgain : 0.2f * p.mgain;
        }
        f32x2 v; v[0] = v0; v[1] = v1;
        *reinterpret_cast<f32x2*>(p.out + o) = v;
    }
}


template <bool ISC>
__global__ __launch_bounds__(WT, 2) void wino6q_kernel(const Wino6Args p) {
    extern __shared__ __attribute__((aligned(16))) unsigned char smem_raw[];
    u32x4* ul = reinterpret_cast<u32x4*>(smem_raw);
    const int tid = threadIdx.x, lane = tid & 63, l31 = lane & 31, half = lane >> 5;
    const int wid = __builtin_amdgcn_readfirstlane(tid >> 6);
    const int grp = wid >> 2, wq = wid & 3, wm = wq >> 1, wrl = wq & 1, gt = tid & (GT - 1);
    unsigned* tl = reinterpret_cast<unsigned*>(smem_raw + U_CHUNKS * 16) + grp * TP_DWORDS;
    const u32x4* tl4 = reinterpret_cast<const u32x4*>(tl);
    int tile, tile_end, tile_step, mbq;
    if (!split6_tile_list(p.ntiles, p.nt8, p.mblocks, p.lists, tile, tile_end, tile_step, mbq)) return;
    const float* inb;
    const float* iscb = nullptr;
    bool has_left, has_right, has_rowout;

    f32x16 acc[2][4];
#pragma unroll
    for (int m = 0; m < 2; ++m)
#pragma unroll
        for (int c = 0; c < 4; ++c)
#pragma unroll
            for (int r = 0; r < 16; ++r) acc[m][c][r] = 0.f;

    unsigned g_off[P_IN];
    int l_off[P_IN], e_flag[P_IN];
    typedef const __attribute__((address_space(4))) Wino6Args* KArgs;
    auto kargs = [&]() {
        KArgs k = (KArgs)__builtin_amdgcn_kernarg_segment_ptr();
        asm volatile("" : "+s"(k));
        return k;
    };
    auto set_tile = [&](int t) {
        const KArgs a = kargs();
        const int aH = a->H, aW = a->W, atx = a->tiles_x, aty = a->tiles_y, aK = a->K;
        const int tx = t % atx, ty = (t / atx) % aty, b = t / (atx * aty);
        const int x0 = tx * TW, yh = ty * TH + PH * grp;
        inb = a->in + (size_t)b * aK * aH * aW;
        if (ISC) iscb = a->isc + (size_t)b * aK;
        has_left = x0 == 0; has_right = x0 + TW == aW; has_rowout = (yh == 0) || (yh + PH == aH);
        int gto = gt;
        asm volatile("" : "+v"(gto));
#pragma unroll
        for (int i = 0; i < P_IN; ++i) {
            const int e = gto + GT * i;
            const int jj = e & 15, q = (e >> 4) & 7, row = e >> 7;
            const int gy = yh - 1 + row;
            const bool left = x0 == 0 && jj == 0, right = x0 + TW == aW && jj == NP - 1, rowout = gy < 0 || gy >= aH;
            e_flag[i] = (left ? 1 : 0) | (right ? 2 : 0) | (rowout ? 4 : 0);
            const int gyc = gy < 0 ? 0 : (gy >= aH ? aH - 1 : gy);
            g_off[i] = (unsigned)((2 * q * aH + gyc) * aW + x0 + 2 * jj - 1 + (left ? 1 : 0) - (right ? 1 : 0));
        }
    };
    set_tile(tile);
#pragma unroll
    for (int i = 0; i < P_IN; ++i) {
        const int e = gt + GT * i;
        const int jj = e & 15, q = (e >> 4) & 7, row = e >> 7;
        l_off[i] = ((row * 2 + (q >> 2)) * NP + jj) * 4 + (q & 3);
    }
    const unsigned q2 = 2u * ((gt >> 4) & 7);
    const size_t plane = (size_t)p.H * p.W;
    const int MT = p.M >> 5;
    f32x4 rin[P_IN][2];
    f32x2 rsc = {1.f, 1.f};
    const int nstage = p.K / KC, nimg = 2 * nstage;
    auto fetch_scales = [&](int s) {
        if (ISC) rsc = *reinterpret_cast<const f32x2u*>(iscb + s * KC + q2);
    };
    auto fetch_item = [&](int i, int s) {
#pragma unroll
        for (int h2 = 0; h2 < 2; ++h2)
            rin[i][h2] = *reinterpret_cast<const f32x4u*>(inb + ((size_t)s * KC + h2) * plane + g_off[i]);
    };
    auto issue_u = [&](int uh, int j) {
        int wqo = wq;
        asm volatile("" : "+s"(wqo));
        const u32x4* us = p.U + ((size_t)(j >> 1) * 36 * MT + 2 * (2 * mbq + (j & 1))) * 64;
        const unsigned pstride = 12u * (unsigned)MT * 64u;
#pragma unroll
        for (int t = 0; t < 3; ++t) {
            const int rem = wqo * 3 + t, kc = (rem >> 1) + 6 * uh, mt = rem & 1;
            const u32x4* g0 = us + (unsigned)(kc * MT + mt) * 64u;
            u32x4* l0 = ul + (kc * 2 + mt) * 64;
#pragma unroll
            for (int piece = 0; piece < 3; ++piece) {
                const u32x4* g = g0 + piece * pstride + (unsigned)lane;
                __builtin_amdgcn_global_load_lds((const __attribute__((address_space(1))) void*)g,
                                                 (__attribute__((address_space(3))) void*)(l0 + piece * 24 * 64), 16, 0, 0);
            }
        }
    };
    unsigned res[P_IN][4][3];
    float te = 0.f, to = 0.f, fe = 0.f, fo = 0.f;
    constexpr int N_SLOT = 3 + 4 * 4 * P_IN;
    auto arith = [&](int k) {
        if (k < 0) {
        } else if (k < P_IN) {
#pragma unroll
            for (int h2 = 0; h2 < 2; ++h2) {
                f32x4 v = rin[k][h2];
                if (has_left) {
                    int f = e_flag[k];
                    asm volatile("" : "+v"(f) :: "memory");
                    if (f & 1) { v[3] = v[2]; v[2] = v[1]; v[1] = v[0]; v[0] = 0.f; }
                }
                if (has_right) {
                    int f = e_flag[k];
                    asm volatile("" : "+v"(f) :: "memory");
                    if (f & 2) { v[0] = v[1]; v[1] = v[2]; v[2] = v[3]; v[3] = 0.f; }
                }
                if (has_rowout) {
                    int f = e_flag[k];
                    asm volatile("" : "+v"(f) :: "memory");
                    if (f & 4) { v[0] = 0.f; v[1] = 0.f; v[2] = 0.f; v[3] = 0.f; }
                }
                rin[k][h2] = ISC ? v * rsc[h2] : v;
                asm volatile("" : "+v"(rin[k][h2]));
            }
        } else if (k < N_SLOT) {
            const int u = (k - P_IN) >> 2, j = (k - P_IN) & 3, i = u >> 2, c = u & 3;
            float ve = 0.f, vo = 0.f;
            if (j == 0) {
                const f32x4 e = rin[i][0], o = rin[i][1];
                ve = c == 0 ? e[0] - e[2] : (c == 1 ? e[1] + e[2] : (c == 2 ? e[2] - e[1] : e[1] - e[3]));
                vo = c == 0 ? o[0] - o[2] : (c == 1 ? o[1] + o[2] : (c == 2 ? o[2] - o[1] : o[1] - o[3]));
            }
            split6_step4(j, ve, vo, te, to, fe, fo, res[i][c][0], res[i][c][1], res[i][c][2]);
        }
    };
    auto write_res = [&]() {
#pragma unroll
        for (int i = 0; i < P_IN; ++i)
#pragma unroll
            for (int c = 0; c < 4; ++c)
#pragma unroll
                for (int pc = 0; pc < 3; ++pc) tl[l_off[i] + (pc * 4 + c) * TP_PLANE] = res[i][c][pc];
    };
    const int rr = l31 >> 4, jj = l31 & 15;
    const int b_chunk = ((2 * wrl + rr) * 2 + half) * NP + jj;
    const int a_chunk = wm * 64 + lane;

    auto multiply = [&](auto mset_tag, int fs) {
        constexpr int MSET = decltype(mset_tag)::value;
        bf16x8 av[2][3], bv[2][3];
        auto rd1 = [&](int g, int slot, int q) {
            const int ky = g >> 2, c = g & 3;
            if (q < 3) av[slot][q] = __builtin_bit_cast(bf16x8, ul[a_chunk + ((q * 3 + ky) * 4 + c) * 128]);
            else bv[slot][q - 3] = __builtin_bit_cast(bf16x8, tl4[b_chunk + (((q - 3) * 4 + c) * PR + ky) * 2 * NP]);
        };
#pragma unroll
        for (int q = 0; q < 6; ++q) rd1(0, 0, q);
        __builtin_amdgcn_s_setprio(1);
#pragma unroll
        for (int g = 0; g < 12; ++g) {
            const int slot = g & 1, c = g & 3;
            if (g == 5) split6_barrier();
            __builtin_amdgcn_sched_barrier(0);
#pragma unroll
            for (int q = 0; q < 6; ++q) {
                split6_product(q, av[slot], bv[slot], acc[MSET][c], acc[MSET][c]);
                if (g + 1 < 12 && q < 3) { rd1(g + 1, slot ^ 1, 2 * q); rd1(g + 1, slot ^ 1, 2 * q + 1); }
                const int k = g * 6 + q;
                if (MSET == 0) {
                    if (k == 5) fetch_scales(fs);
#pragma unroll
                    for (int i = 0; i < P_IN; ++i)
                        if (k == 6 + 12 * i) fetch_item(i, fs);
                } else {
                    arith(k - SLOT0);
                }
                __builtin_amdgcn_sched_barrier(0);
            }
        }
        __builtin_amdgcn_s_setprio(0);
        split6_barrier();
    };
    auto stage = [&](int ph, bool write, bool has_next) {
        const int cs = wino6_sched::renew_image(ph);
        const bool work = wino6_sched::renew_work(cs, nimg, has_next);
        const int ci = cs == nimg ? 0 : cs;
        if (grp == 1 && work) issue_u(1, ci);
        __builtin_amdgcn_sched_barrier(0);
        if (write) write_res();
        if (grp == 1 && work) split6_wait_vm();
        split6_barrier();
        if (grp == 0 && work) {
            issue_u(0, ci);
            split6_wait_vm();
        }
        split6_barrier();
    };

    fetch_scales(0);
#pragma unroll
    for (int i = 0; i < P_IN; ++i) fetch_item(i, 0);
    if (grp == 0) { issue_u(0, 0); issue_u(1, 0); }
#pragma unroll
    for (int k = 0; k < N_SLOT; ++k) arith(k);
    write_res();
    split6_wait_vm();
    split6_barrier();
    for (;;) {
        const bool has_next = tile + tile_step < tile_end;
        int ph = 0;
        if (wino6_sched::lead_phase(grp)) { stage(0, false, has_next); ph = 1; }
        for (int s = 0; s < nstage; ++s) {
            bool next_tile;
            const int fs = wino6_sched::fetch_stage(s, nstage, has_next, next_tile);
            if (next_tile) set_tile(tile + tile_step);
            multiply(std::integral_constant<int, 0>{}, fs);
            stage(ph + 1, false, has_next);
            multiply(std::integral_constant<int, 1>{}, fs);
            if (wino6_sched::runs_sb(grp, s, nstage, has_next)) stage(ph + 3, true, has_next);
            ph += 4;
        }
        for (int i = 0; i < wino6_sched::tail_barriers(grp, has_next); ++i) split6_barrier();

        const KArgs e = kargs();
        const int tx = tile % e->tiles_x, ty = (tile / e->tiles_x) % e->tiles_y, b = tile / (e->tiles_x * e->tiles_y);
        const int x0 = tx * TW, y0 = ty * TH;
        int elane = lane;
        asm volatile("" : "+v"(elane));
        const int ehalf = elane >> 5, err = (elane & 31) >> 4, ejj = elane & 15;
        const int wr = grp * 2 + wrl;
        const int eM = e->M, eW = e->W, eact = e->act;
        const size_t eplane = (size_t)e->H * eW;
        const float emgain = e->mgain;
        const float g_pos = eact == 3 ? 1.4142135623730951f : 1.f;
        float* const eout = e->out;
        const float* const eosc = e->osc; const float* const ebias = e->bias; const float* const eres = e->res; const float* const emref = e->mref;
#pragma unroll
        for (int m = 0; m < 2; ++m) {
            const int mbase = (2 * mbq + m) * BM + wm * 32;
            const size_t off0 = ((size_t)b * eM + mbase) * eplane + (size_t)(y0 + 2 * wr) * eW + x0;
            const unsigned lo = (unsigned)(err * eW + 2 * ejj) + 4u * (unsigned)ehalf * (unsigned)eplane;
#pragma unroll
            for (int r0 = 0; r0 < 16; r0 += 4) {
                float scv[4], biv[4];
#pragma unroll
                for (int r = r0; r < r0 + 4; ++r) {
                    const int mm = mbase + (r & 3) + 8 * (r >> 2) + 4 * ehalf;
                    scv[r - r0] = eosc ? eosc[(size_t)b * eM + mm] : 1.f;
                    biv[r - r0] = ebias ? ebias[mm] : 0.f;
                }
                f32x2 resv[4], mrefv[4];
                if (eres) {
#pragma unroll
                    for (int r = r0; r < r0 + 4; ++r)
                        resv[r - r0] = *reinterpret_cast<const f32x2*>(eres + off0 + (size_t)((r & 3) + 8 * (r >> 2)) * eplane + lo);
                }
                if (emref) {
#pragma unroll
                    for (int r = r0; r < r0 + 4; ++r)
                        mrefv[r - r0] = *reinterpret_cast<const f32x2*>(emref + off0 + (size_t)((r & 3) + 8 * (r >> 2)) * eplane + lo);
                }
#pragma unroll
                for (int r = r0; r < r0 + 4; ++r) {
                    float v0 = acc[m][0][r] + acc[m][1][r] + acc[m][2][r];
                    float v1 = acc[m][1][r] - acc[m][2][r] - acc[m][3][r];
                    const float sc = scv[r - r0], bi = biv[r - r0];
                    v0 = v0 * sc + bi;
                    v1 = v1 * sc + bi;
                    if (eact >= 3) {
                        v0 = (v0 > 0.f ? v0 : v0 * 0.2f) * g_pos;
                        v1 = (v1 > 0.f ? v1 : v1 * 0.2f) * g_pos;
                    }
                    if (eres) { v0 += resv[r - r0][0]; v1 += resv[r - r0][1]; }
                    if (emref) {
                        v0 *= mrefv[r - r0][0] > 0.f ? emgain : 0.2f * emgain;
                        v1 *= mrefv[r - r0][1] > 0.f ? emgain : 0.2f * emgain;
                    }
                    f32x2 v; v[0] = v0; v[1] = v1;
                    *reinterpret_cast<f32x2*>(eout + off0 + (size_t)((r & 3) + 8 * (r >> 2)) * eplane + lo) = v;
                }
            }
        }
        if (!has_next) break;
        tile += tile_step;
#pragma unroll
        for (int m = 0; m < 2; ++m)
#pragma unroll
            for (int c = 0; c < 4; ++c)
#pragma unroll
                for (int r = 0; r < 16; ++r) acc[m][c][r] = 0.f;
    }
}

}

static std::atomic<int> g_w6_form{2};
extern "C" int te_conv_wino6_form(int form) {
    const int old = g_w6_form.load(std::memory_order_relaxed);
    if (form >= 1 && form <= 3) g_w6_form.store(form, std::memory_order_relaxed);
    return old;
}

constexpr int W6_MAX_TPB = 4096;
static std::atomic<int> g_w6_tpb{0};
extern "C" int te_conv_wino6_tiles_per_block(int n) {
    const int old = g_w6_tpb.load(std::memory_order_relaxed);
    if (n >= 0 && n <= W6_MAX_TPB) g_w6_tpb.store(n, std::memory_order_relaxed);
    return old;
}

static int w6_auto_tpb(int nt8c, int mblocks) {
    const int64_t rounds1 = te::cdiv((int64_t)8 * nt8c * mblocks, te::kNumCU);
    for (int n = 4; n >= 2; --n) {
        const int64_t blocks = (int64_t)8 * te::cdiv(nt8c, n) * mblocks;
        if (blocks >= te::kNumCU && te::cdiv(blocks, te::kNumCU) * n <= rounds1) return n;
    }
    return 1;
}

PROF_READBACK(w6p)

extern "C" int te_conv_wino6_supported(int B, int K, int M, int H, int W) {
    if (!(B > 0 && K >= 32 && K % 32 == 0 && M >= BM && M % BM == 0 && H >= TH && H % TH == 0)) return 0;
    const bool wide = W >= TW && W % TW == 0, pair16 = W == 16 && B % 2 == 0;
    if (!wide && !pair16) return 0;
    const int64_t tiles = wide ? (int64_t)B * (H / TH) * (W / TW) : (int64_t)(B / 2) * (H / TH);
    if (!wide && tiles * (M / BM) < te::kNumCU / 2) return 0;
    return ((int64_t)K * H * W * 4 * (wide ? 1 : 2) < 0x7FFFFFFF && tiles * (M / BM) < 0x7FFFFFF0) ? 1 : 0;
}

int te_wino6_launch(float* out, const float* in, const float* U, const float* isc, const float* osc, const float* bias, const float* res,
                    const float* mask_ref, float mask_gain, int act, int B, int K, int M, int H, int W, hipStream_t s) {
    TE_REQUIRE(te_conv_wino6_supported(B, K, M, H, W), TE_ERR_UNSUPPORTED,
               "te_conv_f32(TE_CONV_3X3W6): needs K %% 32 == 0, M %% 64 == 0, W %% 32 == 0 (or W == 16 and an even batch), H %% 8 == 0 (te_conv_wino6_supported)");
    TE_REQUIRE(((reinterpret_cast<uintptr_t>(out) | reinterpret_cast<uintptr_t>(U) | reinterpret_cast<uintptr_t>(res) |
                 reinterpret_cast<uintptr_t>(mask_ref)) & 15) == 0 && (reinterpret_cast<uintptr_t>(in) & 3) == 0, TE_ERR_UNSUPPORTED,
               "te_conv_f32(TE_CONV_3X3W6): 16-byte aligned tensors required");
    Wino6Args a{};
    a.out = out; a.in = in; a.U = reinterpret_cast<const u32x4*>(U); a.isc = isc; a.osc = osc; a.bias = bias; a.res = res;
    a.mref = mask_ref; a.mgain = mask_gain; a.act = act;
    a.B = B; a.K = K; a.M = M; a.H = H; a.W = W;
    a.lgpw = W >= TW ? 4 : 3;
    a.tiles_x = W >= TW ? W / TW : 1; a.tiles_y = H / TH; a.mblocks = M / BM;
    a.ntiles = (W >= TW ? B : B / 2) * a.tiles_x * a.tiles_y;
    a.nt8 = te::xcd_banded() ? (int)te::cdiv(a.ntiles, 8) : 0;
    const int64_t blocks = te::cdiv(a.ntiles, 8) * 8 * a.mblocks;
    const int form = g_w6_form.load(std::memory_order_relaxed);
    const int64_t blocks_q = te::cdiv(a.ntiles, 8) * 8 * (M / (2 * BM));
    if (W >= TW && split6_two_image(form - 1, M, blocks_q)) {
        a.mblocks = M / (2 * BM);
        const int nt8c = (int)te::cdiv(a.ntiles, 8);
        int tpb = g_w6_tpb.load(std::memory_order_relaxed);
        if (tpb == 0) tpb = w6_auto_tpb(nt8c, a.mblocks);
        a.lists = tpb >= 2 ? (int)te::cdiv(nt8c, tpb) : 0;
        const int64_t blocks2 = a.lists ? (int64_t)8 * a.lists * a.mblocks : blocks_q;
        const size_t lds = (size_t)U_CHUNKS * 16 + 2 * (size_t)TP_DWORDS * 4;
        SPLIT6_LAUNCH_ISC(wino6q_kernel, isc, dim3((unsigned)blocks2), WT, lds, s, a);
    } else {
        const size_t lds = (size_t)U_CHUNKS * 16 + 2 * (size_t)TP_DWORDS * 4;
        SPLIT6_LAUNCH_ISC(wino6p_kernel, isc, dim3((unsigned)blocks), WT, lds, s, a);
    }
    return te::launch_status("te_conv_f32(TE_CONV_3X3W6)");
}
```

transeditor_amd/op/modconv.py:

```python
import contextlib

import os

import torch
from torch.autograd import Function

from .. import _lib
from .chanscale import chan_scale
from .fused_act import fused_leaky_relu

import threading


class _Graph:
    __slots__ = ('skip_w',)

    def __init__(self):
        self.skip_w = False


_DEFAULT_GRAPH = _Graph()


class _Local(threading.local):

    def __init__(self):
        self.second_order = False
        self.second_wrt = None
        self.graph = _DEFAULT_GRAPH
        self.frozen_on = False
        self.frozen_cache = None
        self.pack_cache = None

    def __getitem__(self, k):
        if k == 'skip_w':
            return self.graph.skip_w or _DEFAULT_GRAPH.skip_w
        return getattr(self, k)

    def __eq__(self, other):
        return {'second_order': self.second_order, 'skip_w': self['skip_w']} == other


_STATE = _Local()


def current_graph():
    return _STATE.graph if _STATE.second_order else _DEFAULT_GRAPH


@contextlib.contextmanager
def second_order(wrt=None):
    old = (_STATE.second_order, _STATE.graph, _STATE.second_wrt)
    _STATE.second_order, _STATE.graph, _STATE.second_wrt = True, _Graph(), wrt
    try:
        yield _STATE.graph
    finally:
        _STATE.second_order = old[0]
        _STATE.second_wrt = old[2]
        if old[0]:
            _STATE.graph = old[1]


@contextlib.contextmanager
def latent_producer_section():
    if not (_STATE.second_order and _STATE.second_wrt == 'latent'):
        yield
        return
    _STATE.second_order = False
    try:
        yield
    finally:
        _STATE.second_order = True


@contextlib.contextmanager
def no_weight_grads():
    toks = {id(t): t for t in (_STATE.graph, _DEFAULT_GRAPH)}.values()
    old = [(t, t.skip_w) for t in toks]
    for t in toks:
        t.skip_w = True
    try:
        yield
    finally:
        for t, o in old:
            t.skip_w = o


@contextlib.contextmanager
def frozen_weights(cache):
    old = (_STATE.frozen_on, _STATE.frozen_cache)
    _STATE.frozen_on, _STATE.frozen_cache = True, cache
    try:
        yield
    finally:
        _STATE.frozen_on, _STATE.frozen_cache = old


@contextlib.contextmanager
def packed_weights_cache(cache):
    old = _STATE.pack_cache
    _STATE.pack_cache = cache
    try:
        yield
    finally:
        _STATE.pack_cache = old


@contextlib.contextmanager
def cache_of(ctx):
    c = getattr(ctx, 'pack_cache', None)
    if c is None or _STATE.pack_cache is not None:
        yield
        return
    with packed_weights_cache(c):
        yield


def keep_cache(ctx):
    ctx.pack_cache = _STATE.pack_cache


def _pack_key(w, pack_kind, wscale):
    return (w.data_ptr(), tuple(w.shape), pack_kind, float(wscale))


def _cacheable(w):
    if _STATE.pack_cache is None:
        return None
    base = w._base if w._base is not None else w
    return base if isinstance(base, torch.nn.Parameter) else None


def refresh_packed_weights(cache):
    jobs, fresh = [], []
    for key, (ver, wp, base) in list(cache.items()):
        ptr, shape, pack_kind, wscale = key
        if base._version == ver:
            continue
        n = 1
        for d in shape:
            n *= d
        if not (base.data_ptr() == ptr and base.numel() == n and base.is_contiguous() and len(shape) == 4):
            del cache[key]
            continue
        jobs.append((torch.empty_like(wp), base.detach().view(shape), pack_kind, wscale))
        fresh.append((key, base))
    _lib.conv_pack_multi(jobs)
    for (key, base), job in zip(fresh, jobs):
        cache[key] = (base._version, job[0], base)
    return len(jobs)


def packed(w, pack_kind, wscale=1.0):
    base = _cacheable(w)
    if base is None:
        return _lib.conv_pack(w, pack_kind, wscale)
    cache, key = _STATE.pack_cache, _pack_key(w, pack_kind, wscale)
    ent = cache.get(key)
    if ent is None or ent[0] != w._version or ent[2] is not base:
        ent = cache[key] = (w._version, _lib.conv_pack(w, pack_kind, wscale), base)
    return ent[1]


def packed2(w, kind_a, kind_b, wscale=1.0):
    base = _cacheable(w)
    if base is None:
        return _lib.conv_pack2(w, kind_a, kind_b, wscale)
    cache = _STATE.pack_cache
    ka, kb = _pack_key(w, kind_a, wscale), _pack_key(w, kind_b, wscale)
    ea, eb = cache.get(ka), cache.get(kb)
    va = ea is not None and ea[0] == w._version and ea[2] is base
    vb = eb is not None and eb[0] == w._version and eb[2] is base
    if va and vb:
        return ea[1], eb[1]
    if not va and not vb:
        wa, wb = _lib.conv_pack2(w, kind_a, kind_b, wscale)
        cache[ka], cache[kb] = (w._version, wa, base), (w._version, wb, base)
        return wa, wb
    return packed(w, kind_a, wscale), packed(w, kind_b, wscale)


def _frozen_entry(w, kind, wscale, want_wsq, pack_kind=_lib.PACK_FWD):
    base = w._base if w._base is not None else w
    key = (id(base), w.data_ptr(), tuple(w.shape), kind, float(wscale), pack_kind)
    stamp = (base._version, base.data_ptr())
    ent = _STATE.frozen_cache.get(key)
    if ent is None or ent['stamp'] != stamp:
        ent = {'stamp': stamp, 'wp': _lib.conv_pack(w, pack_kind, wscale), 'wsq': None, 'keep': base}
        _STATE.frozen_cache[key] = ent
    if want_wsq and ent['wsq'] is None:
        w3 = w.reshape(w.shape[0], w.shape[1], -1)
        ent['wsq'] = (w3 * wscale).square().sum(dim=2).contiguous()
    return ent


def _modconv_frozen(x, w, isc, osc, bias, act, kind, wscale, demod_eps):
    H, W = _lowres_hw(kind, False, x)
    pk, ck = fwd_kinds(kind, x.shape[0], w, H, W)
    ent = _frozen_entry(w, kind, wscale, demod_eps is not None, pk)
    if demod_eps is not None:
        osc = _lib.demod_from_wsq(ent['wsq'], isc, demod_eps)
    if _rgb_ok(kind, w.shape[0], w.shape[1], x, osc, act):
        return _lib.rgb_fwd(x, w.reshape(w.shape[0], w.shape[1]), isc, bias, wscale)
    return _lib.conv(x, ent['wp'], ck, w.shape[0], H, W, isc, osc, bias, _act_code(act))


_SQRT2 = 2 ** 0.5


def _act_gain(act):
    return _SQRT2 if act is True else float(act)


def _act_code(act):
    if not act:
        return 0
    g = _act_gain(act)
    if abs(g - _SQRT2) < 1e-6:
        return 3
    if abs(g - 1.0) < 1e-6:
        return 4
    raise RuntimeError(f'modconv: leaky-ReLU gain {g} is not one the kernels fuse (sqrt(2) or 1)')


def _lowres_hw(kind, is_output, t):
    H, W = t.shape[2], t.shape[3]
    if (kind == 'up' and is_output) or (kind == 'down' and not is_output):
        if H % 2 == 0 or W % 2 == 0:
            raise RuntimeError(f"kind '{kind}': high-resolution side must be (2H+1)x(2W+1), got {H}x{W}")
        return (H - 1) // 2, (W - 1) // 2
    return H, W


USE_WINOGRAD = True
USE_SPLIT_BF16 = os.environ.get('TE_SPLIT_BF16', '1') != '0'
USE_SPLIT_S2 = os.environ.get('TE_SPLIT_S2', '1') != '0'
USE_SPLIT_T2 = os.environ.get('TE_SPLIT_T2', '1') != '0'
USE_SPLIT_1X1 = os.environ.get('TE_SPLIT_1X1', '1') != '0'

_ROUTES = {
    '3x3': (_lib.CONV_3X3, ((('USE_WINOGRAD', 'USE_SPLIT_BF16'), _lib.wino6_ok, _lib.CONV_3X3W6),
                            (('USE_WINOGRAD',), _lib.wino_ok, _lib.CONV_3X3W))),
    'down': (_lib.CONV_S2, ((('USE_SPLIT_BF16', 'USE_SPLIT_S2'), _lib.s2s6_ok, _lib.CONV_S2S6),)),
    'up': (_lib.CONV_T2, ((('USE_SPLIT_BF16', 'USE_SPLIT_T2'), _lib.t2s6_ok, _lib.CONV_T2S6),)),
    '1x1': (_lib.CONV_1X1, ()),
    'plain1x1': (_lib.CONV_1X1, ((('USE_SPLIT_BF16', 'USE_SPLIT_1X1'), _lib.p1s6_ok, _lib.CONV_1X1S6),)),
}
_ADJOINT = {'3x3': '3x3', 'down': 'up', 'up': 'down', '1x1': '1x1', 'plain1x1': 'plain1x1'}
_PACK = {
    _lib.CONV_3X3: (_lib.PACK_FWD, _lib.PACK_DGRAD), _lib.CONV_1X1: (_lib.PACK_FWD, _lib.PACK_DGRAD),
    _lib.CONV_T2: (_lib.PACK_FWD, _lib.PACK_SWAP), _lib.CONV_S2: (_lib.PACK_FWD, _lib.PACK_SWAP),
    _lib.CONV_3X3W: (_lib.PACK_WFWD, _lib.PACK_WDGRAD), _lib.CONV_3X3W6: (_lib.PACK_W6FWD, _lib.PACK_W6DGRAD),
    _lib.CONV_S2S6: (_lib.PACK_S6FWD, _lib.PACK_S6SWAP), _lib.CONV_T2S6: (_lib.PACK_T6FWD, _lib.PACK_T6SWAP),
    _lib.CONV_1X1S6: (_lib.PACK_P6FWD, _lib.PACK_P6DGRAD),
}


def conv_route(op, B, K, M, H, W, dgrad=False):
    if dgrad:
        op, K, M = _ADJOINT[op], M, K
    ck, preferred = _ROUTES[op]
    switch = globals().__getitem__
    for names, covers, kind in preferred:
        if all(map(switch, names)) and covers(B, K, M, H, W):
            ck = kind
            break
    return _PACK[ck][bool(dgrad)], ck


def fwd_kinds(kind, B, w, H, W):
    return conv_route(kind, B, w.shape[1], w.shape[0], H, W)


def bwd_kinds(kind, B, w, H, W):
    return conv_route(kind, B, w.shape[1], w.shape[0], H, W, dgrad=True)


def plain_1x1_kinds(B, w, H, W, dgrad=False):
    return conv_route('plain1x1', B, w.shape[1], w.shape[0], H, W, dgrad)


def packed_route(op, B, w, H, W, wscale, both):
    K, M = w.shape[1], w.shape[0]
    pk, ck = conv_route(op, B, K, M, H, W)
    if not both:
        return packed(w, pk, wscale), ck, None
    pkb, ckb = conv_route(op, B, K, M, H, W, dgrad=True)
    wp, wpb = packed2(w, pk, pkb, wscale)
    return wp, ck, (wpb, ckb)


def _fwd_raw(x, w, kind, isc=None, osc=None, bias=None, act=0, wscale=1.0, with_bwd_pack=False):
    H, W = _lowres_hw(kind, False, x)
    ahead = _STATE.pack_cache is not None and torch.is_grad_enabled() is False
    wp, ck, bwd = packed_route(kind, x.shape[0], w, H, W, wscale, with_bwd_pack or ahead)
    y = _lib.conv(x, wp, ck, w.shape[0], H, W, isc, osc, bias, act)
    return (y, bwd) if with_bwd_pack else y


def _dgrad_raw(g, w, kind, isc=None, osc=None, wscale=1.0, wp=None):
    H, W = _lowres_hw(kind, True, g)
    if wp is None:
        pk, ck = bwd_kinds(kind, g.shape[0], w, H, W)
        wp = packed(w, pk, wscale)
    else:
        wp, ck = wp
    return _lib.conv(g, wp, ck, w.shape[1], H, W, isc, osc)


def _wgrad_raw(g, x, kind, group=False):
    if kind == 'down':
        H, W = g.shape[2], g.shape[3]
        return _lib.wgrad_slabs(x, g, _lib.CONV_T2, H, W, group)
    H, W = x.shape[2], x.shape[3]
    return _lib.wgrad_slabs(g, x, _ROUTES[kind][0], H, W, group)


def _slab_sum(slabs, kind):
    gw = slabs.sum(dim=(0, 1))
    return gw.transpose(0, 1) if kind == 'down' else gw


def _wgrad_plain(gy, x, kind, ksize, wscale):
    slabs = _wgrad_raw(gy, x, kind, group=True)
    Co, Ci = gy.shape[1], x.shape[1]
    if kind == 'down':
        gw = _slab_sum(slabs, kind)
        gw = gw * wscale if wscale != 1.0 else gw
    else:
        gw, _, _ = _lib.wgrad_reduce(slabs, slabs[0, 0], wscale, None, None, want_w=True)
    return gw.reshape(Co, Ci, ksize, ksize)


class _ConvFwd(Function):
    @staticmethod
    def forward(ctx, x, w, kind, wscale):
        ctx.save_for_backward(x, w)
        ctx.kind, ctx.wscale = kind, wscale
        ctx.graph = current_graph()
        keep_cache(ctx)
        return _fwd_raw(x, w, kind, wscale=wscale)

    @staticmethod
    def backward(ctx, gy):
        x, w = ctx.saved_tensors
        skip_w = ctx.graph.skip_w or _DEFAULT_GRAPH.skip_w
        with cache_of(ctx):
            gx = _ConvDgrad.apply(gy, w, ctx.kind, ctx.wscale) if ctx.needs_input_grad[0] else None
            gw = _ConvWgrad.apply(gy, x, ctx.kind, w.shape[2], ctx.wscale) if (ctx.needs_input_grad[1] and not skip_w) else None
        return gx, gw, None, None


class _ConvDgrad(Function):
    @staticmethod
    def forward(ctx, gy, w, kind, wscale):
        ctx.save_for_backward(gy, w)
        ctx.kind, ctx.wscale = kind, wscale
        keep_cache(ctx)
        return _dgrad_raw(gy, w, kind, wscale=wscale)

    @staticmethod
    def backward(ctx, ggx):
        gy, w = ctx.saved_tensors
        with cache_of(ctx):
            g_gy = _ConvFwd.apply(ggx, w, ctx.kind, ctx.wscale) if ctx.needs_input_grad[0] else None
            g_w = _ConvWgrad.apply(gy, ggx, ctx.kind, w.shape[2], ctx.wscale) if ctx.needs_input_grad[1] else None
        return g_gy, g_w, None, None


class _ConvWgrad(Function):
    @staticmethod
    def forward(ctx, gy, x, kind, ksize, wscale):
        ctx.save_for_backward(gy, x)
        ctx.kind, ctx.wscale = kind, wscale
        keep_cache(ctx)
        return _wgrad_plain(gy, x, kind, ksize, wscale)

    @staticmethod
    def backward(ctx, ggw):
        gy, x = ctx.saved_tensors
        with cache_of(ctx):
            g_gy = _ConvFwd.apply(x, ggw, ctx.kind, ctx.wscale) if ctx.needs_input_grad[0] else None
            g_x = _ConvDgrad.apply(gy, ggw, ctx.kind, ctx.wscale) if ctx.needs_input_grad[1] else None
        return g_gy, g_x, None, None, None


def set_split_bf16(on):
    on = bool(on)
    globals()['USE_SPLIT_BF16'] = on
    _lib.wgrad_split(int(on))
    return on


def conv_core(x, w, kind='3x3', wscale=1.0):
    return _ConvFwd.apply(x, w, kind, float(wscale))


_SCALE_FLOOR = 1e-20


def _nonzero(s):
    if s is None:
        return None
    return _Floor.apply(s)


class _Floor(Function):
    @staticmethod
    def forward(ctx, s):
        return torch.where(s.abs() < _SCALE_FLOOR, torch.where(s < 0, -_SCALE_FLOOR, _SCALE_FLOOR).to(s.dtype), s)

    @staticmethod
    def backward(ctx, g):
        return g


def _rgb_ok(kind, Co, Ci, x_like, osc, act=False):
    return kind == '1x1' and osc is None and not act and _lib.rgb_supported(Co, Ci, x_like.shape[2] * x_like.shape[3])


def _chan_dot(a, b):
    from .chanscale import _ChanDot
    return _ChanDot.apply(a.contiguous(), b.contiguous())


class _MCFwd(Function):
    @staticmethod
    def forward(ctx, x, w, s, d, kind, wscale):
        ctx.kind, ctx.wscale = kind, wscale
        ctx.graph = current_graph()
        keep_cache(ctx)
        if _rgb_ok(kind, w.shape[0], w.shape[1], x, d):
            y = _lib.rgb_fwd(x, w.reshape(3, w.shape[1]), s.contiguous(), None, wscale)
        else:
            y = _fwd_raw(x, w, kind, s.contiguous(), None if d is None else d.contiguous(), None, 0, wscale)
        ctx.save_for_backward(x, w, s, d, y)
        return y

    @staticmethod
    def backward(ctx, gy):
        x, w, s, d, y = ctx.saved_tensors
        need = ctx.needs_input_grad
        skip_w = ctx.graph.skip_w or _DEFAULT_GRAPH.skip_w
        with cache_of(ctx):
            gx = _MCDgrad.apply(gy, w, s, d, ctx.kind, ctx.wscale) if (need[0] or need[2]) else None
            gw = _MCWgrad.apply(gy, x, s, d, ctx.kind, w.shape[2], ctx.wscale) if (need[1] and not skip_w) else None
        gs = _chan_dot(gx, x) / s if need[2] else None
        gd = _chan_dot(gy, y) / d if (d is not None and need[3]) else None
        return (gx if need[0] else None), gw, gs, gd, None, None


class _MCDgrad(Function):
    @staticmethod
    def forward(ctx, gy, w, s, d, kind, wscale):
        ctx.kind, ctx.wscale = kind, wscale
        keep_cache(ctx)
        if _rgb_ok(kind, w.shape[0], w.shape[1], gy, d):
            gx = _lib.rgb_dgrad(gy, w.reshape(3, w.shape[1]), s.contiguous(), w.shape[1], wscale)
        else:
            gx = _dgrad_raw(gy, w, kind, isc=None if d is None else d.contiguous(), osc=s.contiguous(), wscale=wscale)
        ctx.save_for_backward(gy, w, s, d, gx)
        return gx

    @staticmethod
    def backward(ctx, ggx):
        gy, w, s, d, gx = ctx.saved_tensors
        need = ctx.needs_input_grad
        with cache_of(ctx):
            y2 = _MCFwd.apply(ggx, w, s, d, ctx.kind, ctx.wscale) if (need[0] or (d is not None and need[3])) else None
            gw = _MCWgrad.apply(gy, ggx, s, d, ctx.kind, w.shape[2], ctx.wscale) if need[1] else None
        gs = _chan_dot(ggx, gx) / s if need[2] else None
        gd = _chan_dot(gy, y2) / d if (d is not None and need[3]) else None
        return (y2 if need[0] else None), gw, gs, gd, None, None


class _MCWgrad(Function):
    @staticmethod
    def forward(ctx, gy, x, s, d, kind, ksize, wscale):
        ctx.kind, ctx.wscale = kind, wscale
        keep_cache(ctx)
        ctx.save_for_backward(gy, x, s, d)
        Co, Ci = gy.shape[1], x.shape[1]
        gyc, xc = gy.contiguous(), x.contiguous()
        if _rgb_ok(kind, Co, Ci, x, d):
            slabs = _lib.rgb_wgrad_slabs(gyc, xc)
        else:
            slabs = _wgrad_raw(gyc, xc, kind)
        gw, _, _ = _lib.wgrad_reduce(slabs, slabs[0, 0], wscale, s.contiguous(), None if d is None else d.contiguous(), want_w=True)
        return gw.reshape(Co, Ci, ksize, ksize)

    @staticmethod
    def backward(ctx, ggw):
        gy, x, s, d = ctx.saved_tensors
        need = ctx.needs_input_grad
        with cache_of(ctx):
            y2 = _MCFwd.apply(x, ggw, s, d, ctx.kind, ctx.wscale) if (need[0] or (d is not None and need[3])) else None
            gx = _MCDgrad.apply(gy, ggw, s, d, ctx.kind, ctx.wscale) if (need[1] or need[2]) else None
        gs = _chan_dot(gx, x) / s if need[2] else None
        gd = _chan_dot(gy, y2) / d if (d is not None and need[3]) else None
        return (y2 if need[0] else None), (gx if need[1] else None), gs, gd, None, None, None


def _closed_ok(x):
    return x.is_cuda and x.dtype == torch.float32


USE_CLOSED_MODCONV = True


def modconv_closed(x, w, isc, osc, kind='3x3', wscale=1.0):
    return _MCFwd.apply(x, w, _nonzero(isc), _nonzero(osc), kind, float(wscale))


def _composite(x, w, isc, osc, bias, act, kind, wscale=1.0):
    if USE_CLOSED_MODCONV and isc is not None and kind in ('3x3', 'up', '1x1') and _closed_ok(x):
        y = modconv_closed(x, w, isc, osc, kind, wscale)
        if act:
            return fused_leaky_relu(y, bias, 0.2, _act_gain(act))
        return y if bias is None else y + bias[None, :, None, None]
    if isc is not None:
        x = chan_scale(x, isc)
    y = conv_core(x, w, kind, wscale)
    if osc is not None:
        y = chan_scale(y, osc)
    if act:
        return fused_leaky_relu(y, bias, 0.2, _act_gain(act))
    if bias is not None:
        y = y + bias[None, :, None, None]
    return y


class _ModConvFused(Function):
    @staticmethod
    def forward(ctx, x, w, isc, osc, bias, act, kind, wscale, demod_eps):
        ctx.demod = None
        keep_cache(ctx)
        if demod_eps is not None:
            w3 = w.reshape(w.shape[0], w.shape[1], -1)
            osc, wsq = _lib.demod_fwd(w3, isc, wscale, demod_eps)
            ctx.demod = (demod_eps, wsq)
        ctx.rgb = _rgb_ok(kind, w.shape[0], w.shape[1], x, osc, act)
        if ctx.rgb:
            out = _lib.rgb_fwd(x, w.reshape(w.shape[0], w.shape[1]), isc, bias, wscale)
            ctx.save_for_backward(x, w, isc, osc, bias, None)
            ctx.act, ctx.kind, ctx.wscale = act, kind, wscale
            return out
        ctx.stem = (kind == '1x1' and w.shape[1] == 3 and isc is None and osc is None
                    and _lib.rgb_supported(3, w.shape[0], x.shape[2] * x.shape[3]))
        if ctx.stem:
            out = _lib.rgb_expand(x, w.reshape(w.shape[0], 3).t(), bias, _act_code(act), wscale)
            ctx.save_for_backward(x, w, isc, osc, bias, out if act else None)
            ctx.act, ctx.kind, ctx.wscale = act, kind, wscale
            return out
        ctx.wp_bwd = None
        if ctx.needs_input_grad[0]:
            out, ctx.wp_bwd = _fwd_raw(x, w, kind, isc, osc, bias, _act_code(act), wscale, with_bwd_pack=True)
        else:
            out = _fwd_raw(x, w, kind, isc, osc, bias, _act_code(act), wscale)
        ctx.save_for_backward(x, w, isc, osc, bias, out if act else None)
        ctx.act, ctx.kind, ctx.wscale = act, kind, wscale
        return out

    @staticmethod
    def backward(ctx, g):
        with cache_of(ctx):
            return _ModConvFused._backward(ctx, g)

    @staticmethod
    def _backward(ctx, g):
        x, w, isc, osc, bias, out = ctx.saved_tensors
        act, kind, wscale = ctx.act, ctx.kind, ctx.wscale
        need = ctx.needs_input_grad
        if torch.is_grad_enabled():
            with torch.enable_grad():
                al = [None if t is None else t.view_as(t) for t in (x, w, isc, osc, bias)]
                if ctx.demod is not None:
                    from .style import demod as _demod
                    al[3] = _demod(al[1], al[2], wscale, ctx.demod[0])
                    need = tuple(need[:3]) + (False,) + tuple(need[4:])
                y = _composite(al[0], al[1], al[2], al[3], al[4], act, kind, wscale)
                if _DEFAULT_GRAPH.skip_w:
                    need = (need[0], False) + tuple(need[2:])
                ins = [t for t, n in zip(al, need[:5]) if n and t is not None]
                gs = iter(torch.autograd.grad(y, ins, g, create_graph=True, allow_unused=True))
            return tuple(next(gs) if (n and t is not None) else None
                         for t, n in zip(al, need[:5])) + (None, None, None, None)
        g = g.contiguous()
        g_bias = None
        if act:
            g, g_bias = _lib.bias_act_bwd(g, out, 0.2, _act_gain(act), want_bias=bias is not None)
        elif bias is not None and need[4]:
            g_bias = g.sum(dim=(0, 2, 3))
        if getattr(ctx, 'stem', False):
            gx = _lib.rgb_fwd(g, w.reshape(w.shape[0], 3).t().contiguous(), None, None, wscale) if need[0] else None
            gw = None
            if need[1]:
                gw = _lib.rgb_wgrad_slabs(x, g).sum(dim=(0, 1)).reshape(3, w.shape[0]).t().reshape(w.shape)
                gw = gw * wscale if wscale != 1.0 else gw
            return gx, gw, None, None, g_bias, None, None, None, None
# ... 62 lines not shown
```

transeditor_amd/op/styled_rgb.py:

```python
import torch
from torch.autograd import Function

from .. import _lib
from .modconv import _DEFAULT_GRAPH, _composite, _dgrad_raw, _fwd_raw, _wgrad_raw, cache_of, keep_cache

_SQRT2 = 2 ** 0.5


def supported(x, w, wr):
    HW = x.shape[2] * x.shape[3]
    return (x.is_cuda and x.dtype == torch.float32 and w.shape[2] == 3 and wr.shape[0] == 3 and wr.shape[1] == w.shape[0]
            and x.shape[0] <= 64 and w.shape[1] <= 8192 and _lib.rgb_supported(3, w.shape[0], HW))


class _ModConvRGB(Function):
    @staticmethod
    def forward(ctx, x, w, s, bias, wr, sr, br, wscale, eps, wscale_r):
        w3 = w.reshape(w.shape[0], w.shape[1], -1)
        d, wsq = _lib.demod_fwd(w3, s, wscale, eps)
        keep_cache(ctx)
        if ctx.needs_input_grad[0]:
            a, wp_bwd = _fwd_raw(x, w, '3x3', s, d, bias, 3, wscale, with_bwd_pack=True)
        else:
            a, wp_bwd = _fwd_raw(x, w, '3x3', s, d, bias, 3, wscale), None
        rgb = _lib.rgb_fwd(a, wr.reshape(3, wr.shape[1]), sr, br, wscale_r)
        ctx.save_for_backward(x, w, s, bias, wr, sr, br, d, wsq, a)
        ctx.wp_bwd = wp_bwd
        ctx.cfg = (wscale, eps, wscale_r)
        ctx.set_materialize_grads(False)
        return a, rgb

    @staticmethod
    def backward(ctx, ga, grgb):
        with cache_of(ctx):
            return _ModConvRGB._backward(ctx, ga, grgb)

    @staticmethod
    def _backward(ctx, ga, grgb):
        x, w, s, bias, wr, sr, br, d, wsq, a = ctx.saved_tensors
        wscale, eps, wscale_r = ctx.cfg
        need = ctx.needs_input_grad
        if torch.is_grad_enabled():
            with torch.enable_grad():
                from .style import demod as _demod
                al = [t.view_as(t) for t in (x, w, s, bias, wr, sr, br)]
                ac = _composite(al[0], al[1], al[2], _demod(al[1], al[2], wscale, eps), al[3], True, '3x3', wscale)
                rc = _composite(ac, al[4], al[5], None, al[6], False, '1x1', wscale_r)
                outs, gouts = [], []
                if ga is not None:
                    outs.append(ac)
                    gouts.append(ga)
                if grgb is not None:
                    outs.append(rc)
                    gouts.append(grgb)
                nd = list(need[:7])
                if _DEFAULT_GRAPH.skip_w:
                    nd[1] = nd[4] = False
                ins = [t for t, n in zip(al, nd) if n]
                gs = iter(torch.autograd.grad(outs, ins, gouts, create_graph=True, allow_unused=True))
            return tuple(next(gs) if n else None for n in nd) + (None, None, None)
        Co = w.shape[0]
        gwr = gsr = gbr = None
        if grgb is not None:
            grgb = grgb.contiguous()
            if need[6]:
                gbr = grgb.sum(dim=(0, 2, 3))
            if need[4] or need[5]:
                sl = _lib.rgb_wgrad_slabs(grgb, a)
                gwr, gsr, _ = _lib.wgrad_reduce(sl, wr.reshape(3, Co, 1), wscale_r, sr, None, want_w=need[4], want_isc=need[5])
                if gwr is not None:
                    gwr = gwr.reshape(wr.shape)
        if ga is None and grgb is None:
            return (None,) * 10
        if grgb is not None and _lib.bias_act_bwd_rgb_supported(a.shape):
            g, gb = _lib.bias_act_bwd_rgb(ga, a, grgb, wr.reshape(3, Co), sr, wscale_r, 0.2, _SQRT2, want_bias=need[3])
        else:
            gt = ga
            if grgb is not None:
                gr = _lib.rgb_dgrad(grgb, wr.reshape(3, Co), sr, Co, wscale_r)
                gt = gr if gt is None else gt + gr
            g, gb = _lib.bias_act_bwd(gt, a, 0.2, _SQRT2, want_bias=need[3])
        gx = _dgrad_raw(g, w, '3x3', isc=d, osc=s, wscale=wscale, wp=ctx.wp_bwd) if need[0] else None
        gw = gs = None
        if need[1] or need[2]:
            slabs = _wgrad_raw(g, x, '3x3')
            w3 = w.reshape(Co, w.shape[1], -1)
            gw, gs, gd = _lib.wgrad_reduce(slabs, w3, wscale, s, d, want_w=need[1], want_isc=need[2], want_osc=True)
            _lib.demod_bwd(gd, d, w3, wsq, s, wscale, into=(gw, gs))
            if gw is not None:
                gw = gw.reshape(w.shape)
        return gx, gw, gs, gb, gwr, gsr, gbr, None, None, None


def styled_conv_rgb(x, w, s, bias, wr, sr, br, wscale, eps, wscale_r):
    return _ModConvRGB.apply(x, w, s.contiguous(), bias, wr, sr.contiguous(), br, float(wscale), float(eps), float(wscale_r))
```

Baseline: 151.9.

## Fuse ToRGB into Winograd conv epilogue and RGB weight grads into bias-act backward

In the forward pass, the ToRGB 1x1 projection is computed inside the Winograd-6 conv epilogue. Each M-block writes partial RGB sums to a workspace, and a small finish kernel reduces them and adds the bias. This avoids re-reading the activation for a separate rgb_fwd, and a K-split rgb_fwd is used as the fallback. In the backward pass, the bias-act RGB kernel now also accumulates the grgb·ref dot products for the ToRGB weight slabs and the RGB bias sums, so the separate rgb_wgrad_slabs pass and the grgb.sum call are removed. The cost is extra workspace, extra reductions and more register and LDS pressure in the conv and bias-act kernels.

Result: faster. 153.5, median of 6 (+1.0%).

```diff
diff --git a/include/te_hip.h b/include/te_hip.h
--- a/include/te_hip.h
+++ b/include/te_hip.h
@@ -37,6 +37,10 @@
 int te_bias_act_bwd_rgb_f32(float* gi, float* gb, float* ws, const float* g, const float* ref, const float* grgb, const float* wrgb,
                             const float* srgb, float wscale, float alpha, float scale, int64_t outer, int64_t C, int64_t inner,
                             te_stream_t stream);
+int te_bias_act_bwd_rgb_slab_count(int64_t outer, int64_t C, int64_t inner);
+int te_bias_act_bwd_rgb_slabs_f32(float* gi, float* gb, float* ws, float* slabs, float* gbr, float* ws_rgb, const float* g,
+                                  const float* ref, const float* grgb, const float* wrgb, const float* srgb, float wscale,
+                                  float alpha, float scale, int64_t outer, int64_t C, int64_t inner, te_stream_t stream);
 
 int te_upfirdn2d_f32(float* out, const float* x, const float* k, int64_t major, int in_h, int in_w,
                      int minor, int kh, int kw, int up_x, int up_y, int down_x, int down_y, int pad_x0,
@@ -99,6 +103,12 @@
 int te_conv_p1s6_supported(int B, int K, int M, int H, int W);
 int te_conv_wino6_form(int form);
 int te_conv_wino6_tiles_per_block(int n);
+int te_conv_wino6_rgb_supported(int B, int K, int M, int H, int W);
+int64_t te_conv_wino6_rgb_ws_floats(int B, int K, int M, int H, int W);
+int te_conv_wino6_rgb_f32(float* out, float* rgb, float* ws, const float* in, const float* wp, const float* isc, const float* osc,
+                          const float* bias, const float* res, const float* mask_ref, float mask_gain, int act, const float* wrgb,
+                          const float* srgb, const float* brgb, float wscale_rgb, int B, int K, int M, int H, int W,
+                          te_stream_t stream);
 int te_conv_s2s6_form(int form);
 int te_conv_t2s6_form(int form);
 int64_t te_conv_t2s6_ws_floats(int B, int K, int H);
@@ -131,6 +141,9 @@
                    int K, int HW, te_stream_t stream);
 int te_rgb_dgrad_f32(float* gx, const float* g, const float* w, const float* isc, float wscale, int B, int K, int HW,
                      te_stream_t stream);
+int64_t te_rgb_fwd_ws_floats(int B, int K, int HW);
+int te_rgb_fwd_split_f32(float* out, float* ws, const float* x, const float* w, const float* isc, const float* bias, float wscale,
+                         int B, int K, int HW, te_stream_t stream);
 int te_rgb_expand_f32(float* out, const float* x3, const float* w, const float* bias, int act, float wscale, int B, int K,
                       int HW, te_stream_t stream);
 int te_rgb_wgrad_slab_count(int B, int K, int HW);
diff --git a/transeditor_amd/_lib.py b/transeditor_amd/_lib.py
--- a/transeditor_amd/_lib.py
+++ b/transeditor_amd/_lib.py
@@ -176,6 +176,25 @@
 
 
 @_op
+def bias_act_bwd_rgb_slabs(g, ref, grgb, wrgb, srgb, wscale, alpha, scale, want_bias=True, want_rgb_bias=True):
+    ref, grgb = _aligned16(ref.contiguous()), _aligned16(grgb.contiguous())
+    g = _aligned16(g.contiguous()) if g is not None else None
+    gi = torch.empty_like(ref)
+    Bn, Cn, inner = ref.shape[0], ref.shape[1], _inner(ref.shape)
+    gb, ws = _bias_grad_buffers(want_bias, Bn, Cn, inner, ref.device)
+    S = lib().te_bias_act_bwd_rgb_slab_count(Bn, Cn, inner)
+    if S <= 0:
+        raise RuntimeError(f'te_bias_act_bwd_rgb_slabs_f32 does not cover {tuple(ref.shape)} (bias_act_bwd_rgb_supported)')
+    slabs = torch.empty(Bn, S, 3, Cn, 1, device=ref.device, dtype=ref.dtype)
+    gbr = torch.empty(3, device=ref.device, dtype=ref.dtype) if want_rgb_bias else None
+    ws_rgb = torch.empty(3 * Bn * S, device=ref.device, dtype=ref.dtype) if want_rgb_bias else None
+    _launch('te_bias_act_bwd_rgb_slabs_f32', _ptr(gi), _ptr(gb), _ptr(ws), _ptr(slabs), _ptr(gbr), _ptr(ws_rgb), _ptr(g), _ptr(ref),
+            _ptr(grgb), _ptr(wrgb.contiguous()), _ptr(srgb.contiguous()) if srgb is not None else None, wscale, alpha, scale, Bn, Cn,
+            inner)
+    return gi, gb, slabs, gbr
+
+
+@_op
 def upfirdn2d_raw(x, k, up, down, pad, bias=None, act=0, alpha=0.2, scale=1.0):
     x = x.contiguous()
     B, Cn, H, W = x.shape
@@ -311,9 +330,26 @@
     return (B, M, H, W)
 
 
-@_op
-def conv(x, wp, kind, M, H, W, isc=None, osc=None, bias=None, act=0, res=None, mask_ref=None, mask_gain=1.0):
+def conv_rgb_ok(kind, B, K, M, H, W):
+    return kind == CONV_3X3W6 and bool(lib().te_conv_wino6_rgb_supported(B, K, M, H, W))
+
+
+@_op
+def conv(x, wp, kind, M, H, W, isc=None, osc=None, bias=None, act=0, res=None, mask_ref=None, mask_gain=1.0, rgb=None):
     x = x.contiguous()
+    if rgb is not None:
+        wr, sr, br, wscale_r, img = rgb
+        B, K = x.shape[0], x.shape[1]
+        n = lib().te_conv_wino6_rgb_ws_floats(B, K, M, H, W) if kind == CONV_3X3W6 else 0
+        if n <= 0:
+            raise RuntimeError(f'te_hip: no convolution + ToRGB launch for kind {kind} at {B}x{K}->{M}@{H}x{W} (conv_rgb_ok)')
+        if tuple(img.shape) != (B, 3, H, W):
+            raise RuntimeError(f'te_hip: ToRGB image {tuple(img.shape)} does not match the convolution output {(B, 3, H, W)}')
+        out = torch.empty(B, M, H, W, device=x.device, dtype=x.dtype)
+        ws = torch.empty(n, device=x.device, dtype=x.dtype)
+        _launch('te_conv_wino6_rgb_f32', _ptr(out), _ptr(img), _ptr(ws), _ptr(x), _ptr(wp), _ptr(isc), _ptr(osc), _ptr(bias), _ptr(res),
+                _ptr(mask_ref), mask_gain, act, _ptr(wr.contiguous()), _ptr(sr), _ptr(br), wscale_r, B, K, M, H, W)
+        return out
     if kind == CONV_1X1S6:
         x = _aligned16(x)
     res = _aligned16(res.contiguous()) if res is not None else None
@@ -399,11 +435,16 @@
 
 
 @_op
-def rgb_fwd(x, w, isc, bias, wscale=1.0):
+def rgb_fwd(x, w, isc, bias, wscale=1.0, split=False):
     x = _aligned16(x.contiguous())
     B, K, H, W = x.shape
     out = torch.empty(B, 3, H, W, device=x.device, dtype=x.dtype)
-    _launch('te_rgb_fwd_f32', _ptr(out), _ptr(x), _ptr(w.contiguous()), _ptr(isc), _ptr(bias), wscale, B, K, H * W)
+    n = lib().te_rgb_fwd_ws_floats(B, K, H * W) if split else 0
+    if n > 0:
+        ws = torch.empty(n, device=x.device, dtype=x.dtype)
+        _launch('te_rgb_fwd_split_f32', _ptr(out), _ptr(ws), _ptr(x), _ptr(w.contiguous()), _ptr(isc), _ptr(bias), wscale, B, K, H * W)
+    else:
+        _launch('te_rgb_fwd_f32', _ptr(out), _ptr(x), _ptr(w.contiguous()), _ptr(isc), _ptr(bias), wscale, B, K, H * W)
     return out
 
 
diff --git a/transeditor_amd/csrc/bias_act.hip b/transeditor_amd/csrc/bias_act.hip
--- a/transeditor_amd/csrc/bias_act.hip
+++ b/transeditor_amd/csrc/bias_act.hip
@@ -99,12 +99,14 @@
     if (threadIdx.x == 0) gb[blockIdx.x] = acc;
 }
 
+template <bool SLAB>
 __global__ __launch_bounds__(256) void bias_act_bwd_rgb_rows_kernel(float4* __restrict__ gi, float* __restrict__ part,
                                                                     const float4* __restrict__ g, const float4* __restrict__ ref,
                                                                     const float4* __restrict__ grgb, const float* __restrict__ wrgb,
                                                                     const float* __restrict__ srgb, float wscale, float alpha,
-                                                                    float scale, uint32_t C, uint32_t inner4) {
-    __shared__ float lds4[4];
+                                                                    float scale, uint32_t C, uint32_t inner4,
+                                                                    float* __restrict__ slabs = nullptr, float* __restrict__ rpart = nullptr) {
+    __shared__ float lds4[SLAB ? 28 : 4];
     const uint32_t c = blockIdx.y, n = blockIdx.z;
     const size_t row = ((size_t)n * C + c) * inner4;
     const size_t rrow = (size_t)n * 3 * inner4;
@@ -112,6 +114,8 @@
     const float c0 = sc * wrgb[c], c1 = sc * wrgb[C + c], c2 = sc * wrgb[2 * C + c];
     const uint32_t base = blockIdx.x * (256 * kBwdVecPerThread);
     float acc = 0.f;
+    float dot[6] = {0.f, 0.f, 0.f, 0.f, 0.f, 0.f};
+    const bool rsum = SLAB && rpart && c == 0;
 #pragma unroll
     for (int it = 0; it < kBwdVecPerThread; ++it) {
         const uint32_t i = base + it * 256 + threadIdx.x;
@@ -130,9 +134,40 @@
             o.w = gv.w * (rv.w > 0.f ? 1.f : alpha) * scale;
             gi[row + i] = o;
             acc += (o.x + o.y) + (o.z + o.w);
-        }
-    }
-    if (part) {
+            if (SLAB) {
+                dot[0] += (r0.x * rv.x + r0.y * rv.y) + (r0.z * rv.z + r0.w * rv.w);
+                dot[1] += (r1.x * rv.x + r1.y * rv.y) + (r1.z * rv.z + r1.w * rv.w);
+                dot[2] += (r2.x * rv.x + r2.y * rv.y) + (r2.z * rv.z + r2.w * rv.w);
+                if (rsum) {
+                    dot[3] += (r0.x + r0.y) + (r0.z + r0.w);
+                    dot[4] += (r1.x + r1.y) + (r1.z + r1.w);
+                    dot[5] += (r2.x + r2.y) + (r2.z + r2.w);
+                }
+            }
+        }
+    }
+    if (SLAB) {
+        const int lane = threadIdx.x & 63, wid = threadIdx.x >> 6;
+        const int nsum = rsum ? 6 : 3;
+        const float a = part ? wave_sum(acc) : 0.f;
+        if (lane == 0) lds4[wid] = a;
+        for (int q = 0; q < nsum; ++q) {
+            const float d = wave_sum(dot[q]);
+            if (lane == 0) lds4[4 * (q + 1) + wid] = d;
+        }
+        __syncthreads();
+        if (threadIdx.x <= (uint32_t)nsum) {
+            const float* l = lds4 + 4 * threadIdx.x;
+            const float tot = l[0] + l[1] + l[2] + l[3];
+            if (threadIdx.x == 0) {
+                if (part) part[((size_t)c * gridDim.z + n) * gridDim.x + blockIdx.x] = tot;
+            } else if (threadIdx.x <= 3) {
+                slabs[(((size_t)n * gridDim.x + blockIdx.x) * 3 + (threadIdx.x - 1)) * C + c] = tot;
+            } else {
+                rpart[((size_t)(threadIdx.x - 4) * gridDim.z + n) * gridDim.x + blockIdx.x] = tot;
+            }
+        }
+    } else if (part) {
         const float tot = block_sum_256(acc, lds4);
         if (threadIdx.x == 0) part[((size_t)c * gridDim.z + n) * gridDim.x + blockIdx.x] = tot;
     }
@@ -311,8 +346,35 @@
     const uint32_t inner4 = (uint32_t)(inner / 4);
     dim3 grid((unsigned)te::cdiv(inner4, 256 * kBwdVecPerThread), (unsigned)C, (unsigned)outer);
     hipStream_t stream = (hipStream_t)stream_;
-    bias_act_bwd_rgb_rows_kernel<<<grid, 256, 0, stream>>>((float4*)gi, gb ? ws : nullptr, (const float4*)g, (const float4*)ref,
-                                                          (const float4*)grgb, wrgb, srgb, wscale, alpha, scale, (uint32_t)C, inner4);
+    bias_act_bwd_rgb_rows_kernel<false><<<grid, 256, 0, stream>>>((float4*)gi, gb ? ws : nullptr, (const float4*)g, (const float4*)ref,
+                                                                 (const float4*)grgb, wrgb, srgb, wscale, alpha, scale, (uint32_t)C, inner4);
     if (gb) bias_parts_sum_kernel<<<(int)C, 64, 0, stream>>>(gb, ws, (uint32_t)(grid.x * grid.z));
     return te::launch_status("te_bias_act_bwd_rgb_f32");
 }
+
+extern "C" int te_bias_act_bwd_rgb_slab_count(int64_t outer, int64_t C, int64_t inner) {
+    if (!te_bias_act_bwd_rgb_supported(outer, C, inner)) return 0;
+    return (int)te::cdiv(inner / 4, 256 * kBwdVecPerThread);
+}
+
+extern "C" int te_bias_act_bwd_rgb_slabs_f32(float* gi, float* gb, float* ws, float* slabs, float* gbr, float* ws_rgb, const float* g,
+                                             const float* ref, const float* grgb, const float* wrgb, const float* srgb, float wscale,
+                                             float alpha, float scale, int64_t outer, int64_t C, int64_t inner, te_stream_t stream_) {
+    TE_REQUIRE(gi && ref && grgb && wrgb && slabs, TE_ERR_NULL, "te_bias_act_bwd_rgb_slabs_f32: gi/ref/grgb/wrgb/slabs is NULL");
+    TE_REQUIRE(!gb || ws, TE_ERR_NULL, "te_bias_act_bwd_rgb_slabs_f32: the bias gradient needs the workspace (te_bias_act_bwd_ws_floats)");
+    TE_REQUIRE(!gbr || ws_rgb, TE_ERR_NULL,
+               "te_bias_act_bwd_rgb_slabs_f32: the ToRGB bias gradient needs ws_rgb (3 * outer * te_bias_act_bwd_rgb_slab_count floats)");
+    TE_REQUIRE(te_bias_act_bwd_rgb_supported(outer, C, inner), TE_ERR_UNSUPPORTED,
+               "te_bias_act_bwd_rgb_slabs_f32: needs inner %% 4 == 0 and inner >= 1024 (te_bias_act_bwd_rgb_supported)");
+    TE_REQUIRE(te::aligned16(gi) && (!g || te::aligned16(g)) && te::aligned16(ref) && te::aligned16(grgb), TE_ERR_UNSUPPORTED,
+               "te_bias_act_bwd_rgb_slabs_f32: 16-byte aligned tensors required");
+    const uint32_t inner4 = (uint32_t)(inner / 4);
+    dim3 grid((unsigned)te::cdiv(inner4, 256 * kBwdVecPerThread), (unsigned)C, (unsigned)outer);
+    hipStream_t stream = (hipStream_t)stream_;
+    bias_act_bwd_rgb_rows_kernel<true><<<grid, 256, 0, stream>>>((float4*)gi, gb ? ws : nullptr, (const float4*)g, (const float4*)ref,
+                                                                (const float4*)grgb, wrgb, srgb, wscale, alpha, scale, (uint32_t)C, inner4,
+                                                                slabs, gbr ? ws_rgb : nullptr);
+    if (gb) bias_parts_sum_kernel<<<(int)C, 64, 0, stream>>>(gb, ws, (uint32_t)(grid.x * grid.z));
+    if (gbr) bias_parts_sum_kernel<<<3, 64, 0, stream>>>(gbr, ws_rgb, (uint32_t)(grid.x * grid.z));
+    return te::launch_status("te_bias_act_bwd_rgb_slabs_f32");
+}
diff --git a/transeditor_amd/csrc/conv_common.h b/transeditor_amd/csrc/conv_common.h
--- a/transeditor_amd/csrc/conv_common.h
+++ b/transeditor_amd/csrc/conv_common.h
@@ -24,6 +24,8 @@
                    const float* mask_ref, float mask_gain, int act, int B, int K, int M, int H, int W, hipStream_t s);
 int te_wino6_launch(float* out, const float* in, const float* U, const float* isc, const float* osc, const float* bias, const float* res,
                     const float* mask_ref, float mask_gain, int act, int B, int K, int M, int H, int W, hipStream_t s);
+void te_rgb_coef_launch(float* tab, const float* w, const float* isc, float wscale, int B, int M, hipStream_t s);
+void te_rgb_finish_launch(float* out, const float* parts, const float* bias, int nparts, int B, int HW, hipStream_t s);
 int te_s2s6_launch(float* out, const float* in, const float* U, const float* isc, const float* osc, const float* bias, const float* res,
                    const float* mask_ref, float mask_gain, int act, int B, int K, int M, int H, int W, hipStream_t s);
 int te_t2s6_launch(float* out, const float* in, const float* U, const float* isc, const float* osc, const float* bias, int act,
diff --git a/transeditor_amd/csrc/rgb.hip b/transeditor_amd/csrc/rgb.hip
--- a/transeditor_amd/csrc/rgb.hip
+++ b/transeditor_amd/csrc/rgb.hip
@@ -1,4 +1,4 @@
-#include "te_common.h"
+#include "conv_common.h"
 
 namespace {
 
@@ -40,13 +40,65 @@
     }
 }
 
+constexpr int KSPLIT = 64;
+
+__global__ __launch_bounds__(256) void rgb_fwd_split_kernel(float* __restrict__ parts, const float* __restrict__ x,
+                                                            const float* __restrict__ w, const float* __restrict__ isc, float wscale,
+                                                            int K, int HW) {
+    __shared__ float ws[NOUT][KSPLIT];
+    const int b = blockIdx.y, j = blockIdx.z, tid = threadIdx.x;
+    const int k0 = j * KSPLIT, kn = min(KSPLIT, K - k0);
+    if (tid < kn) {
+        const float s = (isc ? isc[(size_t)b * K + k0 + tid] : 1.f) * wscale;
+#pragma unroll
+        for (int o = 0; o < NOUT; ++o) ws[o][tid] = w[o * K + k0 + tid] * s;
+    }
+    __syncthreads();
+    const int HW4 = HW >> 2;
+    const int p4 = blockIdx.x * 256 + tid;
+    if (p4 >= HW4) return;
+    const float4* xp = reinterpret_cast<const float4*>(x + ((size_t)b * K + k0) * HW) + p4;
+    float4 acc[NOUT];
+#pragma unroll
+    for (int o = 0; o < NOUT; ++o) acc[o] = make_float4(0.f, 0.f, 0.f, 0.f);
+#pragma unroll 16
+    for (int k = 0; k < kn; ++k) {
+        const float4 v = xp[(size_t)k * HW4];
+#pragma unroll
+        for (int o = 0; o < NOUT; ++o) {
+            const float c = ws[o][k];
+            acc[o].x += c * v.x; acc[o].y += c * v.y; acc[o].z += c * v.z; acc[o].w += c * v.w;
+        }
+    }
+#pragma unroll
+    for (int o = 0; o < NOUT; ++o)
+        reinterpret_cast<float4*>(parts + (((size_t)j * gridDim.y + b) * NOUT + o) * HW)[p4] = acc[o];
+}
+
+__global__ __launch_bounds__(256) void rgb_finish_kernel(float4* __restrict__ out, const float4* __restrict__ parts,
+                                                         const float* __restrict__ bias, int nparts, uint32_t n4, uint32_t HW4) {
+    const uint32_t i = blockIdx.x * 256 + threadIdx.x;
+    if (i >= n4) return;
+    float4 a = parts[i];
+    for (int j = 1; j < nparts; ++j) {
+        const float4 v = parts[(size_t)j * n4 + i];
+        a.x += v.x; a.y += v.y; a.z += v.z; a.w += v.w;
+    }
+    if (bias) {
+        const float bb = bias[(i / HW4) % NOUT];
+        a.x += bb; a.y += bb; a.z += bb; a.w += bb;
+    }
+    out[i] = a;
+}
+
 __global__ __launch_bounds__(256) void rgb_dgrad_kernel(float* __restrict__ gx, const float* __restrict__ g,
                                                         const float* __restrict__ w, const float* __restrict__ isc,
                                                         float wscale, int K, int HW, const float* __restrict__ bias = nullptr,
-                                                        int act = 0) {
+                                                        int act = 0, int kchunk = KMAX) {
     __shared__ float ws[NOUT][KMAX];
     const int b = blockIdx.y, tid = threadIdx.x;
-    for (int k = tid; k < K; k += 256) {
+    const int k0 = blockIdx.z * kchunk, k1 = min(K, k0 + kchunk);
+    for (int k = k0 + tid; k < k1; k += 256) {
         const float s = (isc ? isc[(size_t)b * K + k] : 1.f) * wscale;
 #pragma unroll
         for (int o = 0; o < NOUT; ++o) ws[o][k] = w[o * K + k] * s;
@@ -61,7 +113,7 @@
     float4* op = reinterpret_cast<float4*>(gx + (size_t)b * K * HW) + p4;
     const float gain = act == 3 ? 1.4142135623730951f : 1.f;
 #pragma unroll 4
-    for (int k = 0; k < K; ++k) {
+    for (int k = k0; k < k1; ++k) {
         const float c0 = ws[0][k], c1 = ws[1][k], c2 = ws[2][k];
         const float bb = bias ? bias[k] : 0.f;
         float4 r;
@@ -179,8 +231,26 @@
     }
 }
 
+__global__ __launch_bounds__(256) void rgb_coef_kernel(float* __restrict__ tab, const float* __restrict__ w,
+                                                       const float* __restrict__ isc, float wscale, int K) {
+    const int b = blockIdx.y, k = blockIdx.x * 256 + threadIdx.x;
+    if (k >= K) return;
+    const float s = (isc ? isc[(size_t)b * K + k] : 1.f) * wscale;
+#pragma unroll
+    for (int o = 0; o < NOUT; ++o) tab[((size_t)b * NOUT + o) * K + k] = w[o * K + k] * s;
+}
+
 inline bool ok_shape(int K, int HW) { return K > 0 && K <= KMAX && HW > 0 && (HW & 3) == 0; }
 
+}
+
+void te_rgb_coef_launch(float* tab, const float* w, const float* isc, float wscale, int B, int M, hipStream_t s) {
+    rgb_coef_kernel<<<dim3((unsigned)te::cdiv(M, 256), (unsigned)B), 256, 0, s>>>(tab, w, isc, wscale, M);
+}
+
+void te_rgb_finish_launch(float* out, const float* parts, const float* bias, int nparts, int B, int HW, hipStream_t s) {
+    const uint32_t n4 = (uint32_t)((int64_t)B * NOUT * HW / 4);
+    rgb_finish_kernel<<<(unsigned)te::cdiv(n4, 256), 256, 0, s>>>((float4*)out, (const float4*)parts, bias, nparts, n4, (uint32_t)(HW / 4));
 }
 
 extern "C" int te_rgb_supported(int M, int K, int HW) { return (M == NOUT && ok_shape(K, HW)) ? 1 : 0; }
@@ -194,12 +264,34 @@
     return te::launch_status("te_rgb_fwd_f32");
 }
 
+extern "C" int64_t te_rgb_fwd_ws_floats(int B, int K, int HW) {
+    if (!(B > 0 && ok_shape(K, HW))) return TE_ERR_SHAPE;
+    const int64_t blocks = te::cdiv(HW / 4, 256) * B;
+    return (blocks < te::kNumCU && K > KSPLIT) ? te::cdiv(K, KSPLIT) * B * NOUT * HW : 0;
+}
+
+extern "C" int te_rgb_fwd_split_f32(float* out, float* ws, const float* x, const float* w, const float* isc, const float* bias,
+                                    float wscale, int B, int K, int HW, te_stream_t stream_) {
+    if (!ws || te_rgb_fwd_ws_floats(B, K, HW) <= 0) return te_rgb_fwd_f32(out, x, w, isc, bias, wscale, B, K, HW, stream_);
+    TE_REQUIRE(out && x && w, TE_ERR_NULL, "te_rgb_fwd_split_f32: NULL pointer");
+    TE_REQUIRE(te::aligned16(out) && te::aligned16(ws) && te::aligned16(x), TE_ERR_UNSUPPORTED,
+               "te_rgb_fwd_split_f32: 16-byte aligned tensors required");
+    const int nparts = (int)te::cdiv(K, KSPLIT);
+    dim3 grid((unsigned)te::cdiv(HW / 4, 256), (unsigned)B, (unsigned)nparts);
+    rgb_fwd_split_kernel<<<grid, 256, 0, (hipStream_t)stream_>>>(ws, x, w, isc, wscale, K, HW);
+    te_rgb_finish_launch(out, ws, bias, nparts, B, HW, (hipStream_t)stream_);
+    return te::launch_status("te_rgb_fwd_split_f32");
+}
+
 extern "C" int te_rgb_dgrad_f32(float* gx, const float* g, const float* w, const float* isc, float wscale, int B, int K,
                                 int HW, te_stream_t stream_) {
     TE_REQUIRE(gx && g && w, TE_ERR_NULL, "te_rgb_dgrad_f32: NULL pointer");
     TE_REQUIRE(B > 0 && ok_shape(K, HW), TE_ERR_UNSUPPORTED, "te_rgb_dgrad_f32: need K <= 512 and H*W %% 4 == 0");
-    dim3 grid((unsigned)te::cdiv(HW / 4, 256), (unsigned)B);
-    rgb_dgrad_kernel<<<grid, 256, 0, (hipStream_t)stream_>>>(gx, g, w, isc, wscale, K, HW);
+    const int64_t blocks = te::cdiv(HW / 4, 256) * B;
+    const int64_t nz = blocks < te::kNumCU ? std::max<int64_t>(1, std::min<int64_t>(te::cdiv(K, 8), te::cdiv(2 * te::kNumCU, blocks))) : 1;
+    const int kchunk = (int)te::cdiv(K, nz);
+    dim3 grid((unsigned)te::cdiv(HW / 4, 256), (unsigned)B, (unsigned)te::cdiv(K, kchunk));
+    rgb_dgrad_kernel<<<grid, 256, 0, (hipStream_t)stream_>>>(gx, g, w, isc, wscale, K, HW, nullptr, 0, kchunk);
     return te::launch_status("te_rgb_dgrad_f32");
 }
 
diff --git a/transeditor_amd/csrc/wino6.hip b/transeditor_amd/csrc/wino6.hip
--- a/transeditor_amd/csrc/wino6.hip
+++ b/transeditor_amd/csrc/wino6.hip
@@ -16,6 +16,7 @@
     int B, K, M, H, W, ntiles, mblocks, tiles_x, tiles_y, nt8;
     int lists;
     int lgpw;
+    const float* rgbc; float* parts;
 };
 
 constexpr int PH = 4, PR = PH + 2;
@@ -271,7 +272,7 @@
 }
 
 
-template <bool ISC>
+template <bool ISC, bool RGB = false>
 __global__ __launch_bounds__(WT, 2) void wino6q_kernel(const Wino6Args p) {
     extern __shared__ __attribute__((aligned(16))) unsigned char smem_raw[];
     u32x4* ul = reinterpret_cast<u32x4*>(smem_raw);
@@ -500,7 +501,11 @@
         const float emgain = e->mgain;
         const float g_pos = eact == 3 ? 1.4142135623730951f : 1.f;
         float* const eout = e->out;
-        const float* const eosc = e->osc; const float* const ebias = e->bias; const float* const eres = e->res; const float* const emref = e->mref;
+        const float* const eosc = e->osc; const float* const ebias = e->bias;
+        const float* const eres = RGB ? nullptr : e->res; const float* const emref = RGB ? nullptr : e->mref;
+        const float* ergbc = nullptr;
+        float prgb[3][2] = {{0.f, 0.f}, {0.f, 0.f}, {0.f, 0.f}};
+        if (RGB) ergbc = e->rgbc + (size_t)b * 3 * eM;
 #pragma unroll
         for (int m = 0; m < 2; ++m) {
             const int mbase = (2 * mbq + m) * BM + wm * 32;
@@ -514,6 +519,15 @@
                     const int mm = mbase + (r & 3) + 8 * (r >> 2) + 4 * ehalf;
                     scv[r - r0] = eosc ? eosc[(size_t)b * eM + mm] : 1.f;
                     biv[r - r0] = ebias ? ebias[mm] : 0.f;
+                }
+                float rgv[3][4];
+                if (RGB) {
+#pragma unroll
+                    for (int r = r0; r < r0 + 4; ++r) {
+                        const int mm = mbase + (r & 3) + 8 * (r >> 2) + 4 * ehalf;
+#pragma unroll
+                        for (int o = 0; o < 3; ++o) rgv[o][r - r0] = ergbc[o * eM + mm];
+                    }
                 }
                 f32x2 resv[4], mrefv[4];
                 if (eres) {
@@ -544,7 +558,29 @@
                     }
                     f32x2 v; v[0] = v0; v[1] = v1;
                     *reinterpret_cast<f32x2*>(eout + off0 + (size_t)((r & 3) + 8 * (r >> 2)) * eplane + lo) = v;
-                }
+                    if (RGB) {
+#pragma unroll
+                        for (int o = 0; o < 3; ++o) {
+                            prgb[o][0] += rgv[o][r - r0] * v0;
+                            prgb[o][1] += rgv[o][r - r0] * v1;
+                        }
+                    }
+                }
+                if (RGB) {
+#pragma unroll
+                    for (int o = 0; o < 3; ++o) asm volatile("" : "+v"(prgb[o][0]), "+v"(prgb[o][1]));
+                }
+            }
+        }
+        if (RGB) {
+            const int j = 2 * mbq + wm;
+            float* const pp = e->parts + ((size_t)j * e->B + b) * 3 * eplane + (size_t)(y0 + 2 * wr + err) * eW + x0 + 2 * ejj;
+#pragma unroll
+            for (int o = 0; o < 3; ++o) {
+                f32x2 v;
+                v[0] = prgb[o][0] + __shfl_xor(prgb[o][0], 32, 64);
+                v[1] = prgb[o][1] + __shfl_xor(prgb[o][1], 32, 64);
+                if (ehalf == 0) *reinterpret_cast<f32x2*>(pp + (size_t)o * eplane) = v;
             }
         }
         if (!has_next) break;
@@ -595,8 +631,15 @@
     return ((int64_t)K * H * W * 4 * (wide ? 1 : 2) < 0x7FFFFFFF && tiles * (M / BM) < 0x7FFFFFF0) ? 1 : 0;
 }
 
-int te_wino6_launch(float* out, const float* in, const float* U, const float* isc, const float* osc, const float* bias, const float* res,
-                    const float* mask_ref, float mask_gain, int act, int B, int K, int M, int H, int W, hipStream_t s) {
+static bool w6_two_image(int B, int M, int H, int W) {
+    if (W < TW) return false;
+    const int64_t ntiles = (int64_t)B * (W / TW) * (H / TH);
+    return split6_two_image(g_w6_form.load(std::memory_order_relaxed) - 1, M, te::cdiv(ntiles, 8) * 8 * (M / (2 * BM)));
+}
+
+static int w6_launch(float* out, const float* in, const float* U, const float* isc, const float* osc, const float* bias, const float* res,
+                     const float* mask_ref, float mask_gain, int act, int B, int K, int M, int H, int W, hipStream_t s,
+                     const float* rgbc, float* parts) {
     TE_REQUIRE(te_conv_wino6_supported(B, K, M, H, W), TE_ERR_UNSUPPORTED,
                "te_conv_f32(TE_CONV_3X3W6): needs K %% 32 == 0, M %% 64 == 0, W %% 32 == 0 (or W == 16 and an even batch), H %% 8 == 0 (te_conv_wino6_supported)");
     TE_REQUIRE(((reinterpret_cast<uintptr_t>(out) | reinterpret_cast<uintptr_t>(U) | reinterpret_cast<uintptr_t>(res) |
@@ -605,6 +648,7 @@
     Wino6Args a{};
     a.out = out; a.in = in; a.U = reinterpret_cast<const u32x4*>(U); a.isc = isc; a.osc = osc; a.bias = bias; a.res = res;
     a.mref = mask_ref; a.mgain = mask_gain; a.act = act;
+    a.rgbc = rgbc; a.parts = parts;
     a.B = B; a.K = K; a.M = M; a.H = H; a.W = W;
     a.lgpw = W >= TW ? 4 : 3;
     a.tiles_x = W >= TW ? W / TW : 1; a.tiles_y = H / TH; a.mblocks = M / BM;
@@ -621,10 +665,48 @@
         a.lists = tpb >= 2 ? (int)te::cdiv(nt8c, tpb) : 0;
         const int64_t blocks2 = a.lists ? (int64_t)8 * a.lists * a.mblocks : blocks_q;
         const size_t lds = (size_t)U_CHUNKS * 16 + 2 * (size_t)TP_DWORDS * 4;
-        SPLIT6_LAUNCH_ISC(wino6q_kernel, isc, dim3((unsigned)blocks2), WT, lds, s, a);
+        if (rgbc) split6_launch<wino6q_kernel<true, true>>(dim3((unsigned)blocks2), WT, lds, s, a);
+        else SPLIT6_LAUNCH_ISC(wino6q_kernel, isc, dim3((unsigned)blocks2), WT, lds, s, a);
     } else {
+        TE_REQUIRE(!rgbc, TE_ERR_UNSUPPORTED, "te_conv_wino6_rgb_f32: the shape does not take the two-image form (te_conv_wino6_rgb_supported)");
         const size_t lds = (size_t)U_CHUNKS * 16 + 2 * (size_t)TP_DWORDS * 4;
         SPLIT6_LAUNCH_ISC(wino6p_kernel, isc, dim3((unsigned)blocks), WT, lds, s, a);
     }
     return te::launch_status("te_conv_f32(TE_CONV_3X3W6)");
 }
+
+int te_wino6_launch(float* out, const float* in, const float* U, const float* isc, const float* osc, const float* bias, const float* res,
+                    const float* mask_ref, float mask_gain, int act, int B, int K, int M, int H, int W, hipStream_t s) {
+    return w6_launch(out, in, U, isc, osc, bias, res, mask_ref, mask_gain, act, B, K, M, H, W, s, nullptr, nullptr);
+}
+
+extern "C" int te_conv_wino6_rgb_supported(int B, int K, int M, int H, int W) {
+    return (te_conv_wino6_supported(B, K, M, H, W) && w6_two_image(B, M, H, W)) ? 1 : 0;
+}
+
+static int64_t w6_rgb_tab_floats(int B, int M) { return te::cdiv((int64_t)B * 3 * M, 4) * 4; }
+
+extern "C" int64_t te_conv_wino6_rgb_ws_floats(int B, int K, int M, int H, int W) {
+    if (!te_conv_wino6_rgb_supported(B, K, M, H, W)) return 0;
+    return w6_rgb_tab_floats(B, M) + (int64_t)(M / 64) * B * 3 * H * W;
+}
+
+extern "C" int te_conv_wino6_rgb_f32(float* out, float* rgb, float* ws, const float* in, const float* wp, const float* isc, const float* osc,
+                                     const float* bias, const float* res, const float* mask_ref, float mask_gain, int act,
+                                     const float* wrgb, const float* srgb, const float* brgb, float wscale_rgb, int B, int K, int M, int H,
+                                     int W, te_stream_t stream_) {
+    TE_REQUIRE(out && rgb && ws && in && wp && isc && wrgb, TE_ERR_NULL, "te_conv_wino6_rgb_f32: out/rgb/ws/in/wp/isc/wrgb is NULL");
+    TE_REQUIRE(!res && !mask_ref, TE_ERR_UNSUPPORTED, "te_conv_wino6_rgb_f32: no residual and no mask stage in this form");
+    TE_REQUIRE(te_conv_wino6_rgb_supported(B, K, M, H, W), TE_ERR_UNSUPPORTED,
+               "te_conv_wino6_rgb_f32: the shape does not take the two-image form (te_conv_wino6_rgb_supported)");
+    TE_REQUIRE(((reinterpret_cast<uintptr_t>(rgb) | reinterpret_cast<uintptr_t>(ws) | reinterpret_cast<uintptr_t>(out) |
+                 reinterpret_cast<uintptr_t>(wp)) & 15) == 0 && (reinterpret_cast<uintptr_t>(in) & 3) == 0, TE_ERR_UNSUPPORTED,
+               "te_conv_wino6_rgb_f32: 16-byte aligned tensors required");
+    hipStream_t s = (hipStream_t)stream_;
+    float* parts = ws + w6_rgb_tab_floats(B, M);
+    te_rgb_coef_launch(ws, wrgb, srgb, wscale_rgb, B, M, s);
+    const int rc = w6_launch(out, in, wp, isc, osc, bias, nullptr, nullptr, mask_gain, act, B, K, M, H, W, s, ws, parts);
+    if (rc) return rc;
+    te_rgb_finish_launch(rgb, parts, brgb, M / 64, B, H * W, s);
+    return te::launch_status("te_conv_wino6_rgb_f32");
+}
diff --git a/transeditor_amd/op/modconv.py b/transeditor_amd/op/modconv.py
--- a/transeditor_amd/op/modconv.py
+++ b/transeditor_amd/op/modconv.py
@@ -290,11 +290,17 @@
     return wp, ck, (wpb, ckb)
 
 
-def _fwd_raw(x, w, kind, isc=None, osc=None, bias=None, act=0, wscale=1.0, with_bwd_pack=False):
+def _fwd_raw(x, w, kind, isc=None, osc=None, bias=None, act=0, wscale=1.0, with_bwd_pack=False, rgb=None):
     H, W = _lowres_hw(kind, False, x)
     ahead = _STATE.pack_cache is not None and torch.is_grad_enabled() is False
     wp, ck, bwd = packed_route(kind, x.shape[0], w, H, W, wscale, with_bwd_pack or ahead)
-    y = _lib.conv(x, wp, ck, w.shape[0], H, W, isc, osc, bias, act)
+    if rgb is not None and isc is not None and _lib.conv_rgb_ok(ck, x.shape[0], w.shape[1], w.shape[0], H, W):
+        img = torch.empty(x.shape[0], 3, H, W, device=x.device, dtype=x.dtype)
+        y = (_lib.conv(x, wp, ck, w.shape[0], H, W, isc, osc, bias, act, rgb=(*rgb, img)), img)
+    else:
+        y = _lib.conv(x, wp, ck, w.shape[0], H, W, isc, osc, bias, act)
+        if rgb is not None:
+            y = (y, None)
     return (y, bwd) if with_bwd_pack else y
 
 
diff --git a/transeditor_amd/op/styled_rgb.py b/transeditor_amd/op/styled_rgb.py
--- a/transeditor_amd/op/styled_rgb.py
+++ b/transeditor_amd/op/styled_rgb.py
@@ -19,11 +19,13 @@
         w3 = w.reshape(w.shape[0], w.shape[1], -1)
         d, wsq = _lib.demod_fwd(w3, s, wscale, eps)
         keep_cache(ctx)
+        torgb = (wr.reshape(3, wr.shape[1]), sr, br, wscale_r)
         if ctx.needs_input_grad[0]:
-            a, wp_bwd = _fwd_raw(x, w, '3x3', s, d, bias, 3, wscale, with_bwd_pack=True)
+            (a, rgb), wp_bwd = _fwd_raw(x, w, '3x3', s, d, bias, 3, wscale, with_bwd_pack=True, rgb=torgb)
         else:
-            a, wp_bwd = _fwd_raw(x, w, '3x3', s, d, bias, 3, wscale), None
-        rgb = _lib.rgb_fwd(a, wr.reshape(3, wr.shape[1]), sr, br, wscale_r)
+            (a, rgb), wp_bwd = _fwd_raw(x, w, '3x3', s, d, bias, 3, wscale, rgb=torgb), None
+        if rgb is None:
+            rgb = _lib.rgb_fwd(a, torgb[0], sr, br, wscale_r, split=True)
         ctx.save_for_backward(x, w, s, bias, wr, sr, br, d, wsq, a)
         ctx.wp_bwd = wp_bwd
         ctx.cfg = (wscale, eps, wscale_r)
@@ -60,19 +62,21 @@
                 gs = iter(torch.autograd.grad(outs, ins, gouts, create_graph=True, allow_unused=True))
             return tuple(next(gs) if n else None for n in nd) + (None, None, None)
         Co = w.shape[0]
-        gwr = gsr = gbr = None
+        gwr = gsr = gbr = sl = None
+        folded = grgb is not None and _lib.bias_act_bwd_rgb_supported(a.shape)
         if grgb is not None:
             grgb = grgb.contiguous()
-            if need[6]:
-                gbr = grgb.sum(dim=(0, 2, 3))
-            if need[4] or need[5]:
-                sl = _lib.rgb_wgrad_slabs(grgb, a)
-                gwr, gsr, _ = _lib.wgrad_reduce(sl, wr.reshape(3, Co, 1), wscale_r, sr, None, want_w=need[4], want_isc=need[5])
-                if gwr is not None:
-                    gwr = gwr.reshape(wr.shape)
+            if not folded:
+                if need[6]:
+                    gbr = grgb.sum(dim=(0, 2, 3))
+                if need[4] or need[5]:
+                    sl = _lib.rgb_wgrad_slabs(grgb, a)
         if ga is None and grgb is None:
             return (None,) * 10
-        if grgb is not None and _lib.bias_act_bwd_rgb_supported(a.shape):
+        if folded and (need[4] or need[5] or need[6]):
+            g, gb, sl, gbr = _lib.bias_act_bwd_rgb_slabs(ga, a, grgb, wr.reshape(3, Co), sr, wscale_r, 0.2, _SQRT2, want_bias=need[3],
+                                                         want_rgb_bias=need[6])
+        elif folded:
             g, gb = _lib.bias_act_bwd_rgb(ga, a, grgb, wr.reshape(3, Co), sr, wscale_r, 0.2, _SQRT2, want_bias=need[3])
         else:
             gt = ga
@@ -80,6 +84,10 @@
                 gr = _lib.rgb_dgrad(grgb, wr.reshape(3, Co), sr, Co, wscale_r)
                 gt = gr if gt is None else gt + gr
             g, gb = _lib.bias_act_bwd(gt, a, 0.2, _SQRT2, want_bias=need[3])
+        if sl is not None and (need[4] or need[5]):
+            gwr, gsr, _ = _lib.wgrad_reduce(sl, wr.reshape(3, Co, 1), wscale_r, sr, None, want_w=need[4], want_isc=need[5])
+            if gwr is not None:
+                gwr = gwr.reshape(wr.shape)
         gx = _dgrad_raw(g, w, '3x3', isc=d, osc=s, wscale=wscale, wp=ctx.wp_bwd) if need[0] else None
         gw = gs = None
         if need[1] or need[2]:
```
